# tanwanirahul/surreal

Hardware: AMD Instinct MI355X
Metric: PPO learner env-steps/sec/node (GAE+update) at 1/2/4/8 GPUs; % HBM roofline (higher is better)
Workload: dtype f32; 1 GPU; C3: synthetic PPO learner batch, reference PPO defaults (LSTM 100, horizon 5, heads 300x200, n_step 25, adapt, z-filter, 10/10 epochs), SawyerLift state dims (obs 42, act 8), 1024 segments split over 1 GPU(s) (1024 per GPU); segments_per_gpu=1024, n_step=25, env_steps_per_learn_per_gpu=25600, global_segments=1024, parallelism=single, epochs_run_last=10, ppo_mode=adapt, launch=hipGraph replay

## Files before the change

### include/surreal_mi.h

```cpp
#ifndef SURREAL_MI_H
#define SURREAL_MI_H

#include <stdint.h>

#ifdef __cplusplus
extern "C" {
#endif

#define SMI_OK            0
#define SMI_E_ARG        -1
#define SMI_E_NOFIT      -2
#define SMI_E_LAUNCH     -3

int         smi_version(void);
const char* smi_last_error(void);

const char* smi_last_launch(void);

int64_t smi_workspace_bytes(void);
int     smi_set_workspace(void* dev_ptr, int64_t bytes);
typedef struct smi_context smi_context;
smi_context* smi_context_create(void* workspace, int64_t bytes);
int          smi_context_make_current(smi_context* ctx);
int          smi_context_destroy(smi_context* ctx);

#define SMI_KT_GEMM_FWD    0
#define SMI_KT_GEMM_DX     1
#define SMI_KT_GEMM_DW     2
#define SMI_KT_GEMM_REDUCE 3
#define SMI_KT_LSTM_FWD    4
#define SMI_KT_LSTM_BWD    5
#define SMI_KT_CNN_FWD     6
#define SMI_KT_CNN_BWD     7
#define SMI_KT_GAE         8
#define SMI_KT_POLICY_STATS 9
#define SMI_KT_POLICY_GRAD 10
#define SMI_KT_VALUE_ROWS  11
#define SMI_KT_ADAM        12
#define SMI_KT_ZF_TMAJOR   13
int smi_kernel_timing(int on);
int smi_kernel_timing_report(int cls, double* out4);

int smi_calib_mfma(int n_wg, int iters, float* out, long long* stamps, void* stream);
int smi_calib_stream(const float* x, float* y, int64_t n, void* stream);
int smi_clock_probe(const int* flag, long long max_ticks, long long* out3, void* stream);
int smi_clock_probe_stop(int* flag, int value, void* stream);

int64_t smi_mlp_param_count(int in_dim, int h1, int h2, int out_dim, int with_log_var);

int64_t smi_ppo_fused_lds_bytes(int rows, int obs_dim, int h1, int h2, int act_dim,
                                int critic_h1, int critic_h2);

int64_t smi_ppo_fused_max_params(void);

int smi_zfilter_apply(const float* x, float* out, int64_t rows, int dim,
                      const float* running_sum, const float* running_sumsq,
                      const float* count, float eps, void* stream);

int smi_zfilter_update(const float* x, int64_t rows, int dim, int64_t row_stride,
                       float* running_sum, float* running_sumsq, float* count,
                       void* stream);

int smi_zfilter_colstats(const float* x, int64_t rows, int dim, int64_t row_stride,
                         float* out_sum, float* out_sumsq, void* stream);

int smi_zfilter_tmajor(const float* obs, const float* obs_next, int B, int T, int S, int D,
                       int use_zf, const float* running_sum, const float* running_sumsq,
                       const float* count, float eps, float* out, int ldo, int form,
                       void* stream);

int smi_reward_filter(float* rewards, int64_t n, float reward_scale, int mode,
                      float* running_sum, float* running_sumsq, float* count,
                      float eps, void* stream);

int smi_reward_filter_partial(float* rewards, int64_t n, float reward_scale, int forward,
                              const float* running_sum, const float* running_sumsq,
                              const float* count, float eps, double* sums3, void* stream);
int smi_reward_filter_commit(const double* sums3, float* running_sum, float* running_sumsq,
                             float* count, void* stream);

int smi_diag_gauss(const float* actions, const float* prob0, const float* prob1,
                   int64_t rows, int act_dim,
                   float* loglik, float* lik, float* kl, float* entropy, void* stream);

int smi_mlp_forward(const float* params, int in_dim, int h1, int h2, int out_dim,
                    int out_act, int with_log_var,
                    const float* x, int64_t rows, int64_t row_stride,
                    int use_zf, const float* zf_sum, const float* zf_sumsq,
                    const float* zf_count, float zf_eps,
                    float* out, void* stream);

int smi_head_forward(const float* params, int in_dim, int h1, int h2, int out_dim, int tanh_out,
                     const float* x, int64_t ldx, int64_t rows, float* ha1, float* ha2,
                     float* y, float* wT, void* stream);
int smi_head_backward_input(const float* params, int in_dim, int h1, int h2, int out_dim,
                            const float* wT, const float* dz, int64_t rows, const float* ha1,
                            const float* ha2, float* dh2, float* dh1, int dx0, int dxn, float* dx,
                            int64_t lddx, const float* mask, int64_t ldm, void* stream);

int smi_ppo_critic_gae(const float* critic_params, int obs_dim, int h1, int h2,
                       int use_zf, const float* zf_sum, const float* zf_sumsq,
                       const float* zf_count, float zf_eps,
                       const float* obs, const float* obs_next,
                       const float* rewards, const float* dones, int B, int T,
                       const float* gamma_tab, const float* lam_tab,
                       float gamma, float gamma_T,
                       float* values, float* adv_raw, float* ret, void* stream);

int smi_gae_windows(const float* values, float* values_masked,
                    const float* rewards, const float* dones,
                    int64_t B, int T, int horizon,
                    const float* gamma_tab, const float* lam_tab,
                    float gamma, float gamma_H,
                    float* adv, float* ret, double* adv_partials,
                    int* n_partials, void* stream);
int smi_gae_windows_max_partials(int64_t B, int T);

int smi_moments(const float* x, int64_t n, const double* partials, int n_partials,
                double* out3, void* stream);

typedef struct smi_ppo_args {
  int B;
  int obs_dim, h1, h2, act_dim;
  int critic_h1, critic_h2;
  int epoch_policy, epoch_baseline;
  int mode;
  int norm_adv;
  int clip_actor_grad, clip_critic_grad;
  int use_zf;
  const float* obs;      int64_t obs_stride;
  const float* actions;  int64_t act_stride;
  const float* behave;   int64_t beh_stride;
  const float* adv_raw;
  const double* adv_moments;
  const float* ret;
  const float* zf_sum;  const float* zf_sumsq;  const float* zf_count;
  const float* rzf_sum; const float* rzf_sumsq; const float* rzf_count;
  float zf_eps;
  float* actor;  const float* ref_actor;  float* critic;
  float* actor_m; float* actor_v; float* critic_m; float* critic_v;
  int* actor_step; int* critic_step;
  const float* hyper;
  double kl_target;
  float kl_cutoff_coeff;
  float actor_max_norm, critic_max_norm;
  float actor_wd, critic_wd;
  float beta1, beta2, adam_eps;
  float* stats;
  float* kl_record; int* kl_count; int kl_capacity;
  int64_t B_global;
  float* xbuf;
  int* dp_state;
  float* adv_out;
} smi_ppo_args;

#define SMI_HYP_CLIP_EPS   0
#define SMI_HYP_BETA       1
#define SMI_HYP_LR_ACTOR   2
#define SMI_HYP_LR_CRITIC  3
#define SMI_HYPX_CLIP_LO   4
#define SMI_HYPX_CLIP_HI   5
#define SMI_HYP_COUNT      6

#define SMI_ST_SURR_LOSS        0
#define SMI_ST_CLIP_SURR_LOSS   1
#define SMI_ST_KL_LOSS_ADAPT    2
#define SMI_ST_ENTROPY          3
#define SMI_ST_POL_KL           4
#define SMI_ST_GRAD_NORM_ACTOR  5
#define SMI_ST_VAL_LOSS         6
#define SMI_ST_VAL_EXPL_VAR     7
#define SMI_ST_GRAD_NORM_CRITIC 8
#define SMI_ST_AVG_RETURN       9
#define SMI_ST_AVG_LOG_SIG     10
#define SMI_ST_AVG_BEHAVE_LIK  11
#define SMI_ST_AVG_IS_WEIGHT   12
#define SMI_ST_REF_BEHAVE_DIFF 13
#define SMI_ST_EPOCHS_RUN      14
#define SMI_ST_POL_KL_ADAPT    15
#define SMI_ST_COUNT           16

int smi_ppo_update_fused(const smi_ppo_args* args, void* stream);

int64_t smi_ppo_xbuf_floats(int obs_dim, int h1, int h2, int act_dim, int critic_h1,
                            int critic_h2, int mode);
int smi_ppo_epoch_grad(const smi_ppo_args* args, int epoch, void* stream);
int smi_ppo_epoch_apply(const smi_ppo_args* args, int epoch, void* stream);

#define SMI_RNN_PH_GAE           0
#define SMI_RNN_PH_PREP          1
#define SMI_RNN_PH_POLICY_FWD    2
#define SMI_RNN_PH_POLICY_BWD    3
#define SMI_RNN_PH_POLICY_APPLY  4
#define SMI_RNN_PH_VALUE_GRAD    5
#define SMI_RNN_PH_VALUE_APPLY   6
#define SMI_RNN_PH_ZSTATS        7
#define SMI_RNN_PH_ZAPPLY        8
#define SMI_RNN_PH_POLICY_DECIDE 9

typedef struct smi_ppo_rnn_args {
  int B, T, horizon;
  int obs_dim, rnn_hidden;
  int h1, h2, act_dim;
  int critic_h1, critic_h2;
  int epoch_policy, epoch_baseline;
  int mode, norm_adv, clip_actor_grad, clip_critic_grad, use_zf;
  int64_t B_global;
  const float* obs;
  const float* obs_next;
  const float* actions;
  const float* rewards;
  const float* dones;
  const float* behave;
  const float* h0;
  const float* c0;
  float* lstm; float* actor; float* critic;
  const float* ref_lstm; const float* ref_actor;
  float* zf_sum; float* zf_sumsq; float* zf_count;
  const float* rzf_sum; const float* rzf_sumsq; const float* rzf_count;
  float zf_eps;
  float* actor_m; float* actor_v; float* critic_m; float* critic_v;
  int* actor_step; int* critic_step;
  const float* hyper;
  const float* gamma_tab; const float* lam_tab;
  float gamma, gamma_H;
  double kl_target;
  float kl_cutoff_coeff, actor_max_norm, critic_max_norm, actor_wd, critic_wd;
  float beta1, beta2, adam_eps;
  float* stats;
  float* kl_record; int* kl_count; int kl_capacity;
  double* moments;
  double* pstat;
  float* xbuf;
  double* zbuf;
  void* scratch; int64_t scratch_bytes;
  int pix_c, pix_h, pix_w, cnn_feat;
  const uint8_t* pixels;
  const uint8_t* pixels_next;
  float* adv_out; float* ret_out;
  int rnn_layer;
  int prep_independent;
} smi_ppo_rnn_args;

#define SMI_RNN_PSTAT 16
int64_t smi_ppo_rnn_scratch_bytes(int B, int T, int horizon, int obs_dim, int rnn_hidden,
                                  int h1, int h2, int act_dim, int critic_h1, int critic_h2,
                                  int pix_c, int pix_h, int pix_w, int cnn_feat, int rnn_layer);
int64_t smi_ppo_rnn_xbuf_floats(int obs_dim, int rnn_hidden, int h1, int h2, int act_dim,
                                int critic_h1, int critic_h2, int pix_c, int pix_h, int pix_w,
                                int cnn_feat, int rnn_layer);
int64_t smi_lstm_param_count(int in_dim, int hidden);
int smi_ppo_rnn_phase(const smi_ppo_rnn_args* args, int phase, int epoch, void* stream);

int smi_lstm_forward(const float* xproj, const float* w_hh, const float* b_hh,
                     const float* h0, const float* c0, int S, int B, int H,
                     float* hbuf, float* cbuf, float* gates_act, void* stream);
int smi_lstm_backward(const float* dh, const float* gates_act, const float* cbuf,
                      const float* w_hh, int S, int B, int H, float* dgates, void* stream);
int smi_lstm_forward_x(const float* x, int64_t ldx, int din, const float* w_ih,
                       const float* b_ih, const float* w_hh, const float* b_hh,
                       const float* h0, const float* c0, int S, int B, int H, float* hbuf,
                       float* cbuf, float* gates_act, float* xproj_scratch, void* stream);

int64_t smi_cnn_param_count(int C, int H, int W, int F);
int64_t smi_cnn_scratch_bytes(int64_t rows, int C, int H, int W, int F);
int smi_cnn_forward(const float* params, const uint8_t* pix, const uint8_t* pix_next, int64_t B,
                    int64_t T, int64_t rows, int C, int H, int W, int F, float* a1, float* a2,
                    float* feat, int64_t ldf, void* stream);
int smi_cnn_backward(const float* params, const uint8_t* pix, const uint8_t* pix_next, int64_t B,
                     int64_t T, int64_t rows, int C, int H, int W, int F, const float* a1,
                     const float* a2, const float* dz, int64_t lddz, float* grad, void* scratch,
                     int64_t scratch_bytes, void* stream);

int smi_zfilter_accumulate(const float* sum_in, const float* sumsq_in, int dim, float rows,
                           float* running_sum, float* running_sumsq, float* count,
                           void* stream);

int smi_adam_clip(float* params, const float* grad, float* m, float* v, int64_t n,
                  int* step, const float* lr_ptr, float beta1, float beta2,
                  float eps, float weight_decay, float max_norm, float clip_value,
                  const int* skip_flag, float* norm_out, void* stream);

int smi_linear_forward(const float* x, int64_t ldx, int rows, int in_dim, const float* w,
                       int64_t ldw, const float* b, int out_dim, int act, float* y, int64_t ldy,
                       void* stream);
int smi_linear_backward_input(const float* dy, int64_t ldg, int rows, int out_dim,
                              const float* w, int64_t ldw, int in_dim, const float* relu_mask,
                              int64_t ldm, float* dx, int64_t lddx, void* stream);
int smi_linear_forward_cat(const float* x, int64_t ldx, int rows, int in_dim, const float* w,
                           int64_t ldw, const float* b, int out_dim, int act, float* y,
                           int64_t ldy, const float* s, int64_t lds, int s_cols, void* stream);
int smi_linear_backward_weight(const float* dy, int64_t ldg, int rows, int out_dim,
                               const float* x, int64_t ldx, int in_dim, float* dw, int64_t lddw,
                               float* db, int accumulate, void* stream);
int smi_dw_group_begin(void);
int smi_dw_group_flush(void* stream);

int smi_mse_grad(const float* q, int64_t q_stride, const float* y, int64_t n, float* dq,
                 float* loss, void* stream);
int smi_neg_mean_grad(const float* q, int64_t q_stride, int64_t n, float* dq, float* loss,
                      void* stream);
int smi_tanh_backward(const float* dy, int64_t ldg, const float* y, int64_t ldy, int64_t rows,
                      int cols, float* dz, int64_t ldz, void* stream);
int smi_copy_cols(const float* src, int64_t lds, int64_t rows, int cols, float* dst,
                  int64_t ldd, void* stream);
int smi_layernorm_forward(const float* x, int64_t ldx, int64_t rows, int n, const float* gamma,
                          const float* beta, float eps, float* y, int64_t ldy, float* mean,
                          float* rstd, void* stream);
int smi_layernorm_backward(const float* dy, int64_t ldg, const float* x, int64_t ldx,
                           const float* mean, const float* rstd, const float* gamma, int64_t rows,
                           int n, int relu_input, float* dx, int64_t lddx, float* dgamma,
                           float* dbeta, void* stream);

int smi_mlp3_forward_stacked(const float* params, int64_t pstride, const int64_t* offsets6,
                             int in_dim, int h1, int h2, int out_dim, int out_act, const float* x,
                             int64_t ldx, int n, float* y, int64_t ldy, void* stream);

int smi_copy_to_host(void* host_dst, const void* src, int64_t nbytes, void* stream);
int smi_copy_gather(void* dst, const void* const* srcs, const int64_t* dst_offsets,
                    const int64_t* nbytes, int n, void* stream);
int smi_soft_update(float* target, const float* src, int64_t n, float tau, void* stream);
int smi_ddpg_stats(const float* actions, int64_t lda, int act_dim, const float* rewards,
                   int64_t rs, const float* y, const float* q, int64_t qs, int64_t n,
                   float* stats4, void* stream);

int smi_ddpg_target(const float* rewards, const float* dones, const float* q_next,
                    const float* q_next2, int64_t n, float gamma_n, float* y,
                    void* stream);

int smi_mt_seed(uint64_t seed, uint32_t* host_state625);
int smi_mt_randint_host(uint32_t* host_state625, int64_t n, int64_t batch,
                        int64_t* out);
int smi_mt_randint(uint32_t* dev_state625, int64_t n, int64_t batch,
                   int64_t* out_indices, void* stream);

int smi_gather_rows(const float* table, int64_t cols, const int64_t* idx,
                    int64_t batch, float* out, void* stream);

#ifdef __cplusplus
}
#endif
#endif
```

### surreal_amd/_lib.py

```python
import contextlib
import threading
import ctypes
import gc
import os

import torch

HERE = os.path.dirname(os.path.abspath(__file__))
_VARIANT = os.environ.get('SMI_LIB_VARIANT')
LIB_PATH = os.path.join(HERE, 'libsurreal_mi.so' if not _VARIANT else f'libsurreal_mi_{_VARIANT}.so')

c_int, c_i64, c_f32, c_f64, c_vp = ctypes.c_int, ctypes.c_int64, ctypes.c_float, ctypes.c_double, ctypes.c_void_p
P = ctypes.c_void_p

HYP_CLIP_EPS, HYP_BETA, HYP_LR_ACTOR, HYP_LR_CRITIC, HYP_CLIP_LO, HYP_CLIP_HI, HYP_COUNT = range(7)
ST_NAMES = ['_surr_loss', '_clip_surr_loss', '_kl_loss_adapt', '_entropy', '_pol_kl',
            'grad_norm_actor', '_val_loss', '_val_explained_var', 'grad_norm_critic',
            '_avg_return_targ', '_avg_log_sig', '_avg_behave_likelihood', '_avg_is_weight',
            '_ref_behave_diff', 'epochs_run', '_pol_kl_adapt']
ST_COUNT = len(ST_NAMES)
ST = {n: i for i, n in enumerate(ST_NAMES)}


class PPOArgs(ctypes.Structure):
    _fields_ = [
        ('B', c_int), ('obs_dim', c_int), ('h1', c_int), ('h2', c_int), ('act_dim', c_int),
        ('critic_h1', c_int), ('critic_h2', c_int),
        ('epoch_policy', c_int), ('epoch_baseline', c_int),
        ('mode', c_int), ('norm_adv', c_int),
        ('clip_actor_grad', c_int), ('clip_critic_grad', c_int), ('use_zf', c_int),
        ('obs', P), ('obs_stride', c_i64),
        ('actions', P), ('act_stride', c_i64),
        ('behave', P), ('beh_stride', c_i64),
        ('adv_raw', P), ('adv_moments', P), ('ret', P),
        ('zf_sum', P), ('zf_sumsq', P), ('zf_count', P),
        ('rzf_sum', P), ('rzf_sumsq', P), ('rzf_count', P),
        ('zf_eps', c_f32),
        ('actor', P), ('ref_actor', P), ('critic', P),
        ('actor_m', P), ('actor_v', P), ('critic_m', P), ('critic_v', P),
        ('actor_step', P), ('critic_step', P),
        ('hyper', P),
        ('kl_target', c_f64), ('kl_cutoff_coeff', c_f32),
        ('actor_max_norm', c_f32), ('critic_max_norm', c_f32),
        ('actor_wd', c_f32), ('critic_wd', c_f32),
        ('beta1', c_f32), ('beta2', c_f32), ('adam_eps', c_f32),
        ('stats', P),
        ('kl_record', P), ('kl_count', P), ('kl_capacity', c_int),
        ('B_global', c_i64), ('xbuf', P), ('dp_state', P),
        ('adv_out', P),
    ]


class RNNArgs(ctypes.Structure):
    _fields_ = [
        ('B', c_int), ('T', c_int), ('horizon', c_int), ('obs_dim', c_int), ('rnn_hidden', c_int),
        ('h1', c_int), ('h2', c_int), ('act_dim', c_int), ('critic_h1', c_int), ('critic_h2', c_int),
        ('epoch_policy', c_int), ('epoch_baseline', c_int),
        ('mode', c_int), ('norm_adv', c_int), ('clip_actor_grad', c_int), ('clip_critic_grad', c_int),
        ('use_zf', c_int),
        ('B_global', c_i64),
        ('obs', P), ('obs_next', P), ('actions', P), ('rewards', P), ('dones', P), ('behave', P),
        ('h0', P), ('c0', P),
        ('lstm', P), ('actor', P), ('critic', P), ('ref_lstm', P), ('ref_actor', P),
        ('zf_sum', P), ('zf_sumsq', P), ('zf_count', P),
        ('rzf_sum', P), ('rzf_sumsq', P), ('rzf_count', P),
        ('zf_eps', c_f32),
        ('actor_m', P), ('actor_v', P), ('critic_m', P), ('critic_v', P),
        ('actor_step', P), ('critic_step', P),
        ('hyper', P), ('gamma_tab', P), ('lam_tab', P),
        ('gamma', c_f32), ('gamma_H', c_f32),
        ('kl_target', c_f64),
        ('kl_cutoff_coeff', c_f32), ('actor_max_norm', c_f32), ('critic_max_norm', c_f32),
        ('actor_wd', c_f32), ('critic_wd', c_f32),
        ('beta1', c_f32), ('beta2', c_f32), ('adam_eps', c_f32),
        ('stats', P), ('kl_record', P), ('kl_count', P), ('kl_capacity', c_int),
        ('moments', P), ('pstat', P), ('xbuf', P), ('zbuf', P),
        ('scratch', P), ('scratch_bytes', c_i64),
        ('pix_c', c_int), ('pix_h', c_int), ('pix_w', c_int), ('cnn_feat', c_int),
        ('pixels', P), ('pixels_next', P),
        ('adv_out', P), ('ret_out', P),
        ('rnn_layer', c_int), ('prep_independent', c_int),
    ]


RNN_PH_GAE, RNN_PH_PREP, RNN_PH_POLICY_FWD, RNN_PH_POLICY_BWD, RNN_PH_POLICY_APPLY, \
    RNN_PH_VALUE_GRAD, RNN_PH_VALUE_APPLY, RNN_PH_ZSTATS, RNN_PH_ZAPPLY, RNN_PH_POLICY_DECIDE = range(10)
RNN_PSTAT = 16
KT_NAMES = ['gemm_fwd', 'gemm_dx', 'gemm_dw', 'gemm_splitk_reduce', 'lstm_fwd', 'lstm_bwd',
            'cnn_fwd', 'cnn_bwd',
            'gae', 'policy_rows_stats', 'policy_rows_grad', 'value_rows', 'adam', 'zf_tmajor']
KT_BYTES = set(KT_NAMES[8:])


def kernel_timing(on):
    check(lib().smi_kernel_timing(1 if on else 0), 'smi_kernel_timing')


def kernel_timing_report():
    out = {}
    buf = (c_f64 * 4)()
    for i, n in enumerate(KT_NAMES):
        check(lib().smi_kernel_timing_report(i, ctypes.cast(buf, P)), 'smi_kernel_timing_report')
        if buf[0] > 0:
            out[n] = (int(buf[0]), float(buf[1]), float(buf[2]))
    return out

_SIGS = {
    'smi_version': (c_int, []),
    'smi_last_error': (ctypes.c_char_p, []),
    'smi_last_launch': (ctypes.c_char_p, []),
    'smi_workspace_bytes': (c_i64, []),
    'smi_set_workspace': (c_int, [P, c_i64]),
    'smi_context_create': (P, [P, c_i64]),
    'smi_context_make_current': (c_int, [P]),
    'smi_context_destroy': (c_int, [P]),
    'smi_mlp_param_count': (c_i64, [c_int, c_int, c_int, c_int, c_int]),
    'smi_ppo_fused_lds_bytes': (c_i64, [c_int] * 7),
    'smi_ppo_fused_max_params': (c_i64, []),
    'smi_zfilter_apply': (c_int, [P, P, c_i64, c_int, P, P, P, c_f32, P]),
    'smi_zfilter_update': (c_int, [P, c_i64, c_int, c_i64, P, P, P, P]),
    'smi_zfilter_colstats': (c_int, [P, c_i64, c_int, c_i64, P, P, P]),
    'smi_zfilter_tmajor': (c_int, [P, P, c_int, c_int, c_int, c_int, c_int, P, P, P, c_f32, P,
                                   c_int, c_int, P]),
    'smi_reward_filter': (c_int, [P, c_i64, c_f32, c_int, P, P, P, c_f32, P]),
    'smi_reward_filter_partial': (c_int, [P, c_i64, c_f32, c_int, P, P, P, c_f32, P, P]),
    'smi_reward_filter_commit': (c_int, [P, P, P, P, P]),
    'smi_dw_group_begin': (c_int, []),
    'smi_dw_group_flush': (c_int, [P]),
    'smi_layernorm_forward': (c_int, [P, c_i64, c_i64, c_int, P, P, c_f32, P, c_i64, P, P, P]),
    'smi_layernorm_backward': (c_int, [P, c_i64, P, c_i64, P, P, P, c_i64, c_int, c_int, P, c_i64,
                                       P, P, P]),
    'smi_diag_gauss': (c_int, [P, P, P, c_i64, c_int, P, P, P, P, P]),
    'smi_mlp_forward': (c_int, [P, c_int, c_int, c_int, c_int, c_int, c_int, P, c_i64, c_i64,
                                c_int, P, P, P, c_f32, P, P]),
    'smi_ppo_critic_gae': (c_int, [P, c_int, c_int, c_int, c_int, P, P, P, c_f32, P, P, P, P,
                                   c_int, c_int, P, P, c_f32, c_f32, P, P, P, P]),
    'smi_gae_windows': (c_int, [P, P, P, P, c_i64, c_int, c_int, P, P, c_f32, c_f32, P, P, P,
                                P, P]),
    'smi_gae_windows_max_partials': (c_int, [c_i64, c_int]),
    'smi_moments': (c_int, [P, c_i64, P, c_int, P, P]),
    'smi_ppo_update_fused': (c_int, [ctypes.POINTER(PPOArgs), P]),
    'smi_ppo_xbuf_floats': (c_i64, [c_int] * 7),
    'smi_ppo_epoch_grad': (c_int, [ctypes.POINTER(PPOArgs), c_int, P]),
    'smi_ppo_epoch_apply': (c_int, [ctypes.POINTER(PPOArgs), c_int, P]),
    'smi_zfilter_accumulate': (c_int, [P, P, c_int, c_f32, P, P, P, P]),
    'smi_adam_clip': (c_int, [P, P, P, P, c_i64, P, P, c_f32, c_f32, c_f32, c_f32, c_f32, c_f32,
                              P, P, P]),
    'smi_linear_forward': (c_int, [P, c_i64, c_int, c_int, P, c_i64, P, c_int, c_int, P, c_i64, P]),
    'smi_linear_forward_cat': (c_int, [P, c_i64, c_int, c_int, P, c_i64, P, c_int, c_int, P, c_i64,
                                       P, c_i64, c_int, P]),
    'smi_linear_backward_input': (c_int, [P, c_i64, c_int, c_int, P, c_i64, c_int, P, c_i64, P,
                                          c_i64, P]),
    'smi_linear_backward_weight': (c_int, [P, c_i64, c_int, c_int, P, c_i64, c_int, P, c_i64, P,
                                           c_int, P]),
    'smi_mse_grad': (c_int, [P, c_i64, P, c_i64, P, P, P]),
    'smi_neg_mean_grad': (c_int, [P, c_i64, c_i64, P, P, P]),
    'smi_tanh_backward': (c_int, [P, c_i64, P, c_i64, c_i64, c_int, P, c_i64, P]),
    'smi_copy_cols': (c_int, [P, c_i64, c_i64, c_int, P, c_i64, P]),
    'smi_mlp3_forward_stacked': (c_int, [P, c_i64, P, c_int, c_int, c_int, c_int, c_int, P, c_i64,
                                         c_int, P, c_i64, P]),
    'smi_copy_to_host': (c_int, [P, P, c_i64, P]),
    'smi_copy_gather': (c_int, [P, P, P, P, c_int, P]),
    'smi_head_forward': (c_int, [P, c_int, c_int, c_int, c_int, c_int, P, c_i64, c_i64, P, P, P, P,
                                 P]),
    'smi_head_backward_input': (c_int, [P, c_int, c_int, c_int, c_int, P, P, c_i64, P, P, P, P,
                                        c_int, c_int, P, c_i64, P, c_i64, P]),
    'smi_soft_update': (c_int, [P, P, c_i64, c_f32, P]),
    'smi_ddpg_stats': (c_int, [P, c_i64, c_int, P, c_i64, P, P, c_i64, c_i64, P, P]),
    'smi_ddpg_target': (c_int, [P, P, P, P, c_i64, c_f32, P, P]),
    'smi_mt_seed': (c_int, [ctypes.c_uint64, P]),
    'smi_mt_randint_host': (c_int, [P, c_i64, c_i64, P]),
    'smi_mt_randint': (c_int, [P, c_i64, c_i64, P, P]),
    'smi_gather_rows': (c_int, [P, c_i64, P, c_i64, P, P]),
    'smi_lstm_param_count': (c_i64, [c_int, c_int]),
    'smi_kernel_timing': (c_int, [c_int]),
    'smi_kernel_timing_report': (c_int, [c_int, P]),
    'smi_calib_mfma': (c_int, [c_int, c_int, P, P, P]),
    'smi_calib_stream': (c_int, [P, P, c_i64, P]),
    'smi_clock_probe': (c_int, [P, ctypes.c_longlong, P, P]),
    'smi_clock_probe_stop': (c_int, [P, c_int, P]),
    'smi_ppo_rnn_scratch_bytes': (c_i64, [c_int] * 15),
    'smi_ppo_rnn_xbuf_floats': (c_i64, [c_int] * 12),
    'smi_cnn_param_count': (c_i64, [c_int] * 4),
    'smi_cnn_scratch_bytes': (c_i64, [c_i64] + [c_int] * 4),
    'smi_cnn_forward': (c_int, [P, P, P, c_i64, c_i64, c_i64] + [c_int] * 4 + [P, P, P, c_i64, P]),
    'smi_cnn_backward': (c_int, [P, P, P, c_i64, c_i64, c_i64] + [c_int] * 4 +
                         [P, P, P, c_i64, P, P, c_i64, P]),
    'smi_ppo_rnn_phase': (c_int, [ctypes.POINTER(RNNArgs), c_int, c_int, P]),
    'smi_lstm_forward': (c_int, [P, P, P, P, P, c_int, c_int, c_int, P, P, P, P]),
    'smi_lstm_backward': (c_int, [P, P, P, P, c_int, c_int, c_int, P, P]),
    'smi_lstm_forward_x': (c_int, [P, c_i64, c_int, P, P, P, P, P, P, c_int, c_int, c_int,
                                   P, P, P, P, P]),
}

_lib = None


def lib():
    global _lib
    if _lib is None:
        if not os.path.exists(LIB_PATH):
            raise RuntimeError('libsurreal_mi.so not built: run `python -c "import __graft_entry__ as '
                               'g; g.build()"` (no CPU fallback exists)')
        L = ctypes.CDLL(LIB_PATH)
        for name, (res, args) in _SIGS.items():
            fn = getattr(L, name)
            fn.restype = res
            fn.argtypes = args
        _lib = L
    return _lib


def exported_symbols():
    return list(_SIGS)


def check(rc, name):
    if rc != 0:
        msg = lib().smi_last_error().decode(errors='replace')
        raise RuntimeError(f'{name} failed (rc={rc}): {msg}')


def call(name, *args):
    rc = getattr(lib(), name)(*args)
    check(rc, name)
    return rc


def ptr(t):
    if t is None:
        return None
    if not t.is_cuda:
        raise RuntimeError('surreal_amd kernels take device (HIP) tensors; got a CPU tensor '
                           '(there is no CPU fallback)')
    return ctypes.c_void_p(t.data_ptr())


def stream(device=None):
    return ctypes.c_void_p(torch.cuda.current_stream(device).cuda_stream)


_workspaces = {}


def ensure_workspace(device):
    dev = torch.device(device)
    key = dev.index if dev.index is not None else torch.cuda.current_device()
    if key not in _workspaces:
        nbytes = lib().smi_workspace_bytes()
        ws = torch.zeros(nbytes // 4, dtype=torch.float32, device=dev)
        _workspaces[key] = ws
        check(lib().smi_set_workspace(ctypes.c_void_p(ws.data_ptr()), nbytes), 'smi_set_workspace')
    return _workspaces[key]


_ctx_tls = threading.local()


class Context(object):

    def __init__(self, device):
        self.device = torch.device(device)
        nbytes = lib().smi_workspace_bytes()
        self.ws = torch.zeros(nbytes // 4, dtype=torch.float32, device=self.device)
        self.handle = lib().smi_context_create(ctypes.c_void_p(self.ws.data_ptr()), nbytes)
        if not self.handle:
            check(-1, 'smi_context_create')

    def make_current(self):
        check(lib().smi_context_make_current(ctypes.c_void_p(self.handle)), 'smi_context_make_current')
        _ctx_tls.current = self

    def __del__(self):
        h, self.handle = getattr(self, 'handle', None), None
        if h and _lib is not None:
            _lib.smi_context_destroy(ctypes.c_void_p(h))


@contextlib.contextmanager
def gc_paused():
    was = gc.isenabled()
    gc.disable()
    try:
        yield
    finally:
        if was:
            gc.enable()


def require_gpu():
    if not torch.cuda.is_available():
        raise RuntimeError('surreal_amd requires an AMD GPU (HIP); none is visible and there is '
                           'no CPU fallback')
```

### surreal_amd/csrc/linear_kernels.hip

```cpp
#include <cmath>
#include <algorithm>
#include <stdlib.h>
#include <type_traits>
#include "smi_device.hpp"
#include "smi_internal.hpp"
#include "lstm_cell.hpp"

namespace smi {

enum { EPI_FWD = 0, EPI_DX = 1, EPI_DW = 2 };

constexpr int GBM = 64, GBN = 64, GBK = 32;
constexpr int LD_KC = 36;
constexpr int LD_RC = 80;
constexpr int G_STAGE = 2560;

struct GemmArgs {
  int M, N, K;
  const float* A; int64_t a_rs, a_cs;
  const float* B; int64_t b_rs, b_cs;
  float* C; int64_t ldc;
  const float* bias;
  int act;
  const float* mask; int64_t ldm;
  int accumulate;
  int ones_col;
  float* bias_out;
  int kchunk;
  float* part;
  const int* skip;
  int avec, bvec;
  const float* B2; int64_t b2_rs; int split_col, c1_real;
  float* C2; int64_t ldc2; float* bias_out2;
  const float* xsrc; int64_t xlds; int xcols;
};

__device__ __forceinline__ float dw_put(const GemmArgs& g, int m, int n, float v) {
  if (n == g.ones_col) {
    const float b = g.accumulate ? g.bias_out[m] + v : v;
    g.bias_out[m] = b;
    if (g.bias_out2) {
      const float b2 = g.accumulate ? g.bias_out2[m] + v : v;
      g.bias_out2[m] = b2;
      return b * b + b2 * b2;
    }
    return b * b;
  }
  float* dst;
  if (g.B2 && n >= g.split_col) dst = g.C2 + (int64_t)m * g.ldc2 + (n - g.split_col);
  else if (g.B2 && n >= g.c1_real) return 0.f;
  else dst = g.C + (int64_t)m * g.ldc + n;
  const float r = g.accumulate ? *dst + v : v;
  *dst = r;
  return r * r;
}

struct TileRegs { float v[8]; };

struct TileIdx { int mt, nt, z; };
__device__ __forceinline__ TileIdx gemm_tile_index() {
  const int gm = gridDim.x, gn = gridDim.y;
  const int nwg = gm * gn * gridDim.z;
  const int orig = blockIdx.x + gm * (blockIdx.y + gn * blockIdx.z);
  int w = orig;
  if (nwg > 8) {
    const int x = orig & 7, q = nwg >> 3, r = nwg & 7;
    w = (x < r ? x * (q + 1) : r * (q + 1) + (x - r) * q) + (orig >> 3);
  }
  TileIdx t;
  t.nt = w % gn;
  t.mt = (w / gn) % gm;
  t.z = w / (gn * gm);
  return t;
}

template <bool KCONTIG>
__device__ __forceinline__ void gemm_load(const float* __restrict__ P, int64_t rs, int64_t cs,
                                          int r0, int rdata, int k0, int kmax, int ones_col,
                                          bool vec, TileRegs& t) {
  if (vec && ones_col < 0 && r0 + 64 <= rdata && k0 + 32 <= kmax) {
    const float* base = KCONTIG ? P + (int64_t)r0 * rs + k0 : P + (int64_t)k0 * cs + r0;
#pragma unroll
    for (int j = 0; j < 2; ++j) {
      const int q = threadIdx.x + j * kWG;
      const float* src = KCONTIG ? base + (int64_t)(q >> 3) * rs + ((q & 7) << 2)
                                 : base + (int64_t)(q >> 4) * cs + ((q & 15) << 2);
      const float4 x = *reinterpret_cast<const float4*>(src);
      t.v[4 * j + 0] = x.x; t.v[4 * j + 1] = x.y; t.v[4 * j + 2] = x.z; t.v[4 * j + 3] = x.w;
    }
    return;
  }
  if (vec) {
#pragma unroll
    for (int j = 0; j < 2; ++j) {
      const int q = threadIdx.x + j * kWG;
      if (KCONTIG) {
        const int r = q >> 3, k = (q & 7) << 2;
        const int rr = r0 + r, kk = k0 + k;
        const int rc = rr < rdata ? rr : rdata - 1;
        const int kc = kk < kmax ? kk : kmax - 4;
        const float4 x = *reinterpret_cast<const float4*>(P + (int64_t)rc * rs + kc);
        const bool ok = rr < rdata && kk < kmax;
        t.v[4 * j + 0] = ok ? x.x : 0.f; t.v[4 * j + 1] = ok ? x.y : 0.f;
        t.v[4 * j + 2] = ok ? x.z : 0.f; t.v[4 * j + 3] = ok ? x.w : 0.f;
      } else {
        const int k = q >> 4, r = (q & 15) << 2;
        const int rr = r0 + r, kk = k0 + k;
        const int rc = rr < rdata ? rr : rdata - 4;
        const int kc = kk < kmax ? kk : kmax - 1;
        const float4 x = *reinterpret_cast<const float4*>(P + (int64_t)kc * cs + rc);
        const bool okk = kk < kmax, ok = okk && rr < rdata;
        t.v[4 * j + 0] = ok ? x.x : 0.f; t.v[4 * j + 1] = ok ? x.y : 0.f;
        t.v[4 * j + 2] = ok ? x.z : 0.f; t.v[4 * j + 3] = ok ? x.w : 0.f;
        if (ones_col >= 0 && okk) {
#pragma unroll
          for (int e = 0; e < 4; ++e)
            if (rr + e == ones_col) t.v[4 * j + e] = 1.f;
        }
      }
    }
    return;
  }
#pragma unroll
  for (int j = 0; j < 8; ++j) {
    const int idx = threadIdx.x + j * kWG;
    const int r = KCONTIG ? (idx >> 5) : (idx & 63);
    const int k = KCONTIG ? (idx & 31) : (idx >> 6);
    const int rr = r0 + r, kk = k0 + k;
    const int rc = rr < rdata ? rr : rdata - 1;
    const int kc = kk < kmax ? kk : kmax - 1;
    const float x = P[(int64_t)rc * rs + (int64_t)kc * cs];
    t.v[j] = (rr < rdata && kk < kmax) ? x : 0.f;
    if (ones_col >= 0 && rr == ones_col && kk < kmax) t.v[j] = 1.f;
  }
}

template <bool KCONTIG>
__device__ __forceinline__ void gemm_store(float* __restrict__ S, bool vec, const TileRegs& t) {
  if (vec) {
#pragma unroll
    for (int j = 0; j < 2; ++j) {
      const int q = threadIdx.x + j * kWG;
      const float4 x = float4{t.v[4 * j], t.v[4 * j + 1], t.v[4 * j + 2], t.v[4 * j + 3]};
      if (KCONTIG) {
        const int r = q >> 3, k = (q & 7) << 2;
        *reinterpret_cast<float4*>(S + r * LD_KC + k) = x;
      } else {
        const int k = q >> 4, r = (q & 15) << 2;
        *reinterpret_cast<float4*>(S + k * LD_RC + r) = x;
      }
    }
    return;
  }
#pragma unroll
  for (int j = 0; j < 8; ++j) {
    const int idx = threadIdx.x + j * kWG;
    const int r = KCONTIG ? (idx >> 5) : (idx & 63);
    const int k = KCONTIG ? (idx & 31) : (idx >> 6);
    if (KCONTIG) S[r * LD_KC + k] = t.v[j];
    else S[k * LD_RC + r] = t.v[j];
  }
}

template <int EPI, bool AK, bool BK>
__global__ void __launch_bounds__(kWG)
gemm_kernel(GemmArgs g) {
  if (g.skip && g.skip[0] != 0) return;
  __shared__ __attribute__((aligned(16))) float sA[2][G_STAGE];
  __shared__ __attribute__((aligned(16))) float sB[2][G_STAGE];
  const int tid = threadIdx.x, lane = tid & 63, wave = tid >> 6;
  const int li = lane & 15, lk = lane >> 4;
  const TileIdx ti = gemm_tile_index();
  const int m0 = ti.mt * GBM, n0 = ti.nt * GBN;
  const int kb = ti.z * g.kchunk;
  const int ke = min(g.K, kb + g.kchunk);
  const int nk = (ke - kb + GBK - 1) / GBK;
  f32x4 tot[4];
#pragma unroll
  for (int c = 0; c < 4; ++c) tot[c] = f32x4{0.f, 0.f, 0.f, 0.f};
  TileRegs ra[2], rb[2];
  const int bdata = g.ones_col >= 0 ? g.ones_col : g.N;
  if (nk > 0) {
    gemm_load<AK>(g.A, g.a_rs, g.a_cs, m0, g.M, kb, ke, -1, g.avec, ra[0]);
    gemm_load<BK>(g.B, g.b_cs, g.b_rs, n0, bdata, kb, ke, g.ones_col, g.bvec, rb[0]);
  }
  if (nk > 1) {
    gemm_load<AK>(g.A, g.a_rs, g.a_cs, m0, g.M, kb + GBK, ke, -1, g.avec, ra[1]);
    gemm_load<BK>(g.B, g.b_cs, g.b_rs, n0, bdata, kb + GBK, ke, g.ones_col, g.bvec, rb[1]);
  }
  if (nk > 0) {
    gemm_store<AK>(sA[0], g.avec, ra[0]);
    gemm_store<BK>(sB[0], g.bvec, rb[0]);
  }
  __syncthreads();
  const int ar = wave * 16 + li;
  auto kstep = [&](int kt, auto cur_c) {
    constexpr int cur = decltype(cur_c)::value;
    if (kt + 2 < nk) {
      gemm_load<AK>(g.A, g.a_rs, g.a_cs, m0, g.M, kb + (kt + 2) * GBK, ke, -1, g.avec, ra[cur]);
      gemm_load<BK>(g.B, g.b_cs, g.b_rs, n0, bdata, kb + (kt + 2) * GBK, ke, g.ones_col, g.bvec,
                    rb[cur]);
    }
    const float* As = sA[cur];
    const float* Bs = sB[cur];
    f32x4 acc[4];
#pragma unroll
    for (int c = 0; c < 4; ++c) acc[c] = f32x4{0.f, 0.f, 0.f, 0.f};
    float av[8], bv[4][8];
#pragma unroll
    for (int u = 0; u < 8; ++u) {
      const int k = 4 * u + lk;
      av[u] = AK ? As[ar * LD_KC + k] : As[k * LD_RC + ar];
#pragma unroll
      for (int c = 0; c < 4; ++c) {
        const int n = c * 16 + li;
        bv[c][u] = BK ? Bs[n * LD_KC + k] : Bs[k * LD_RC + n];
      }
    }
#pragma unroll
    for (int u = 0; u < 8; ++u)
#pragma unroll
      for (int c = 0; c < 4; ++c) acc[c] = mfma4(av[u], bv[c][u], acc[c]);
#pragma unroll
    for (int c = 0; c < 4; ++c) tot[c] += acc[c];
    if (kt + 1 < nk) {
      gemm_store<AK>(sA[cur ^ 1], g.avec, ra[cur ^ 1]);
      gemm_store<BK>(sB[cur ^ 1], g.bvec, rb[cur ^ 1]);
    }
    __syncthreads();
  };
  for (int kt = 0; kt < nk; kt += 2) {
    kstep(kt, std::integral_constant<int, 0>{});
    if (kt + 1 < nk) kstep(kt + 1, std::integral_constant<int, 1>{});
  }
#pragma unroll
  for (int c = 0; c < 4; ++c) {
    const int n = n0 + c * 16 + li;
    if (n >= g.N) continue;
    float bias_n = 0.f;
    if constexpr (EPI == EPI_FWD) bias_n = g.bias ? g.bias[n] : 0.f;
#pragma unroll
    for (int i = 0; i < 4; ++i) {
      const int m = m0 + wave * 16 + lk * 4 + i;
      if (m >= g.M) continue;
      float v = tot[c][i];
      if constexpr (EPI == EPI_FWD) {
        if (g.part) {
          g.part[((int64_t)ti.z * g.M + m) * g.N + n] = v;
          continue;
        }
        v += bias_n;
        if (g.act == ACT_RELU) v = v > 0.f ? v : 0.f;
        else if (g.act == ACT_TANH) v = tanhf(v);
        g.C[(int64_t)m * g.ldc + n] = v;
      } else if constexpr (EPI == EPI_DX) {
        if (g.part) {
          g.part[((int64_t)ti.z * g.M + m) * g.N + n] = v;
          continue;
        }
        if (g.mask) v = g.mask[(int64_t)m * g.ldm + n] > 0.f ? v : 0.f;
        g.C[(int64_t)m * g.ldc + n] = v;
      } else {
        if (g.part) {
          g.part[((int64_t)ti.z * g.M + m) * g.N + n] = v;
        } else if (n == g.ones_col) {
          g.bias_out[m] = g.accumulate ? g.bias_out[m] + v : v;
        } else {
          float* dst = g.C + (int64_t)m * g.ldc + n;
          *dst = g.accumulate ? *dst + v : v;
        }
      }
    }
  }
}

constexpr int DWD_ZMAX = 8192;
__device__ __attribute__((aligned(16))) float g_dwd_zero[DWD_ZMAX];
__device__ __attribute__((aligned(16))) float g_dwd_one[4] = {1.f, 0.f, 0.f, 0.f};

__global__ void __launch_bounds__(kWG)
gemm_splitk_reduce_kernel(const float* __restrict__ part, int S, GemmArgs g, const float* bias,
                          int act, const float* mask) {
  if (g.skip && g.skip[0] != 0) return;
  __shared__ float red[4][64];
  const int M = g.M, N = g.N;
  const int64_t MN = (int64_t)M * N;
  const int el = threadIdx.x & 63, zl = threadIdx.x >> 6;
  const int64_t e = (int64_t)blockIdx.x * 64 + el;
  const int64_t ec = e < MN ? e : MN - 1;
  float s0 = 0.f, s1 = 0.f, s2 = 0.f, s3 = 0.f;
  int z = zl;
  if (S <= 64) {
    const float* pz = part + (int64_t)zl * MN + ec;
    const int64_t st4 = 4 * MN;
    float v[16];
#pragma unroll
    for (int k = 0; k < 16; ++k) v[k] = *(zl + 4 * k < S ? pz + k * st4 : g_dwd_zero);
#pragma unroll
    for (int k = 0; k < 16; ++k) asm volatile("" : "+v"(v[k]));
    const int nfull = S > zl + 12 ? (S - zl - 12 + 15) / 16 : 0;
#pragma unroll
    for (int j = 0; j < 4; ++j) {
      if (j < nfull) {
        s0 += v[4 * j]; s1 += v[4 * j + 1]; s2 += v[4 * j + 2]; s3 += v[4 * j + 3];
      }
    }
#pragma unroll
    for (int k = 0; k < 16; ++k)
      if (k >= 4 * nfull && zl + 4 * k < S) s0 += v[k];
    z = S;
  }
  for (; z + 12 < S; z += 16) {
    s0 += part[(int64_t)z * MN + ec];
    s1 += part[(int64_t)(z + 4) * MN + ec];
    s2 += part[(int64_t)(z + 8) * MN + ec];
    s3 += part[(int64_t)(z + 12) * MN + ec];
  }
  for (; z < S; z += 4) s0 += part[(int64_t)z * MN + ec];
  red[zl][el] = (s0 + s1) + (s2 + s3);
  __syncthreads();
  if (zl != 0 || e >= MN) return;
  float s = (red[0][el] + red[1][el]) + (red[2][el] + red[3][el]);
  const int m = (int)(e / N), n = (int)(e - (int64_t)m * N);
  if (bias) s += bias[n];
  if (act == ACT_RELU) s = s > 0.f ? s : 0.f;
  else if (act == ACT_TANH) s = tanhf(s);
  if (mask && !(mask[(int64_t)m * g.ldm + n] > 0.f)) s = 0.f;
  dw_put(g, m, n, s);
}

template <int NKU>
__global__ void __launch_bounds__(kWG)
gemm_smallk_fwd_kernel(const float* __restrict__ X, int64_t ldx, int M, int K,
                       const float* __restrict__ W, int64_t ldw, const float* __restrict__ bias,
                       int N, int act, float* __restrict__ Y, int64_t ldy, const int* skip) {
  if (skip && skip[0] != 0) return;
  extern __shared__ __attribute__((aligned(16))) float sW[];
  constexpr int LDK = 4 * NKU + 1;
  constexpr int LDO = 68;
  float* sb = sW + N * LDK;
  float* so = sb + ((N + 3) & ~3) + (threadIdx.x >> 6) * 16 * LDO;
  {
    const int tot = N * LDK;
    for (int e0 = threadIdx.x; e0 < tot; e0 += 8 * kWG) {
      float v[8];
#pragma unroll
      for (int j = 0; j < 8; ++j) {
        const int e = e0 + j * kWG;
        const int ec = e < tot ? e : tot - 1;
        const int n = ec / LDK, k = ec - n * LDK;
        const float x = W[(int64_t)n * ldw + (k < K ? k : K - 1)];
        v[j] = k < K ? x : 0.f;
      }
#pragma unroll
      for (int j = 0; j < 8; ++j) {
        const int e = e0 + j * kWG;
        if (e < tot) sW[e] = v[j];
      }
    }
  }
  for (int n = threadIdx.x; n < N; n += kWG) sb[n] = bias ? bias[n] : 0.f;
  __syncthreads();
  const int lane = threadIdx.x & 63, wave = threadIdx.x >> 6, li = lane & 15, lk = lane >> 4;
  const bool vec_out = ((reinterpret_cast<uintptr_t>(Y) & 15) == 0) && (ldy % 4 == 0);
  for (int tile = blockIdx.x; tile * 64 < M; tile += gridDim.x) {
    const int m = tile * 64 + wave * 16 + li;
    const int mc = m < M ? m : M - 1;
    float a[NKU];
#pragma unroll
    for (int u = 0; u < NKU; ++u) {
      const int k = 4 * u + lk;
      const float x = X[(int64_t)mc * ldx + (k < K ? k : K - 1)];
      a[u] = k < K ? x : 0.f;
    }
    for (int nb = 0; nb < N; nb += 64) {
      f32x4 acc[4];
      const float* w[4];
#pragma unroll
      for (int c = 0; c < 4; ++c) {
        acc[c] = f32x4{0.f, 0.f, 0.f, 0.f};
        const int n = nb + c * 16 + li;
        w[c] = sW + (n < N ? n : N - 1) * LDK + lk;
      }
      float bw[4][NKU];
#pragma unroll
      for (int c = 0; c < 4; ++c)
#pragma unroll
        for (int u = 0; u < NKU; ++u) bw[c][u] = w[c][4 * u];
#pragma unroll
      for (int u = 0; u < NKU; ++u)
#pragma unroll
        for (int c = 0; c < 4; ++c) acc[c] = mfma4(a[u], bw[c][u], acc[c]);
#pragma unroll
      for (int c = 0; c < 4; ++c) {
        const int col = nb + c * 16 + li;
        const float bn = col < N ? sb[col] : 0.f;
#pragma unroll
        for (int i = 0; i < 4; ++i) {
          float v = acc[c][i] + bn;
          if (act == ACT_RELU) v = v > 0.f ? v : 0.f;
          else if (act == ACT_TANH) v = tanhf(v);
          so[(lk * 4 + i) * LDO + c * 16 + li] = v;
        }
      }
      __builtin_amdgcn_wave_barrier();
#pragma unroll
      for (int j = 0; j < 4; ++j) {
        const int r = j * 4 + (lane >> 4), c4 = (lane & 15) * 4;
        const int row = tile * 64 + wave * 16 + r, col = nb + c4;
        const float4 v = *reinterpret_cast<const float4*>(so + r * LDO + c4);
        if (row < M) {
          float* dst = Y + (int64_t)row * ldy + col;
          if (vec_out && col + 3 < N) {
            *reinterpret_cast<float4*>(dst) = v;
          } else {
            if (col < N) dst[0] = v.x;
            if (col + 1 < N) dst[1] = v.y;
            if (col + 2 < N) dst[2] = v.z;
            if (col + 3 < N) dst[3] = v.w;
          }
        }
      }
      __builtin_amdgcn_wave_barrier();
    }
  }
}

static int launch_smallk_fwd(const float* X, int64_t ldx, int M, int K, const float* W,
                             int64_t ldw, const float* b, int N, int act, float* Y, int64_t ldy,
                             hipStream_t st, const int* skip) {
  const int nku = (K + 3) / 4 <= 4 ? 4 : (K + 3) / 4 <= 8 ? 8 : (K + 3) / 4 <= 12 ? 12 : 16;
  const size_t lds = ((size_t)N * (4 * nku + 1) + ((N + 3) & ~3) + 4 * 16 * 68) * 4;
  const int tiles = (M + 63) / 64;
  const int kslot = ktime_begin(st);
  const char* form = "gemm_smallk_fwd_kernel";
#define SMI_SK_CASE(V)                                                                         \
  if (nku == V) {                                                                              \
    form = "gemm_smallk_fwd_kernel<" #V ">";                                                   \
    auto k = gemm_smallk_fwd_kernel<V>;                                                        \
    allow_lds(k, lds);                                                                         \
    static int cap = 0;                                                                        \
    if (!cap) cap = resident_grid(k, kWG, lds);                                                \
    const int grid = tiles < cap ? tiles : cap;                                                \
    hipLaunchKernelGGL(k, dim3(grid), dim3(kWG), lds, st, X, ldx, M, K, W, ldw, b, N, act, Y, \
                       ldy, skip);                                                             \
  }
  SMI_SK_CASE(4) SMI_SK_CASE(8) SMI_SK_CASE(12) SMI_SK_CASE(16)
#undef SMI_SK_CASE
  ktime_end(kslot, KT_GEMM_FWD, 2.0 * M * (double)N * K, st);
  return check_launch(form);
}

constexpr int D2_T = 128, D2_LD = 144;

__device__ __forceinline__ void dw2_load(const float* __restrict__ P, int64_t rs, int c0,
                                         int cdata, int ones_col, int k0, int kmax, float4 (&r)[4]) {
#pragma unroll
  for (int j = 0; j < 4; ++j) {
    const int q = threadIdx.x + j * kWG;
    const int k = q >> 5, c = c0 + ((q & 31) << 2);
    const int kk = k0 + k;
    const int kc = kk < kmax ? kk : kmax - 1;
    const int cc = c + 3 < cdata ? c : (cdata >= 4 ? cdata - 4 : 0);
    float4 v = *reinterpret_cast<const float4*>(P + (int64_t)kc * rs + cc);
    const bool okk = kk < kmax;
    v.x = okk && c < cdata ? v.x : 0.f;
    v.y = okk && c + 1 < cdata ? v.y : 0.f;
    v.z = okk && c + 2 < cdata ? v.z : 0.f;
    v.w = okk && c + 3 < cdata ? v.w : 0.f;
    if (ones_col >= 0 && okk) {
      if (c == ones_col) v.x = 1.f;
      if (c + 1 == ones_col) v.y = 1.f;
      if (c + 2 == ones_col) v.z = 1.f;
      if (c + 3 == ones_col) v.w = 1.f;
    }
    r[j] = v;
  }
}

__device__ __forceinline__ void dw2_store(float* __restrict__ S, const float4 (&r)[4]) {
#pragma unroll
  for (int j = 0; j < 4; ++j) {
    const int q = threadIdx.x + j * kWG;
    *reinterpret_cast<float4*>(S + (q >> 5) * D2_LD + ((q & 31) << 2)) = r[j];
  }
}

__global__ void __launch_bounds__(kWG)
gemm_dw128_kernel(GemmArgs g) {
  if (g.skip && g.skip[0] != 0) return;
  __shared__ __attribute__((aligned(16))) float sA[2][32 * D2_LD];
  __shared__ __attribute__((aligned(16))) float sB[2][32 * D2_LD];
  const int tid = threadIdx.x, lane = tid & 63, wave = tid >> 6;
  const int li = lane & 15, lk = lane >> 4;
  const TileIdx ti = gemm_tile_index();
  const int m0 = ti.mt * D2_T, n0 = ti.nt * D2_T;
  const int kb = ti.z * g.kchunk;
  const int ke = min(g.K, kb + g.kchunk);
  const int nk = (ke - kb + 31) / 32;
  const int bdata = g.ones_col >= 0 ? g.ones_col + 1 : g.N;
  const int bload = g.ones_col >= 0 ? g.ones_col : g.N;
  f32x4 acc[2][8];
#pragma unroll
  for (int a = 0; a < 2; ++a)
#pragma unroll
    for (int b = 0; b < 8; ++b) acc[a][b] = f32x4{0.f, 0.f, 0.f, 0.f};
  float4 ra[4], rb[4];
  (void)bdata;
  if (nk > 0) {
    dw2_load(g.A, g.a_cs, m0, g.M, -1, kb, ke, ra);
    dw2_load(g.B, g.b_rs, n0, bload, g.ones_col, kb, ke, rb);
    dw2_store(sA[0], ra);
    dw2_store(sB[0], rb);
  }
  __syncthreads();
  for (int kt = 0; kt < nk; ++kt) {
    const int cur = kt & 1;
    if (kt + 1 < nk) {
      dw2_load(g.A, g.a_cs, m0, g.M, -1, kb + (kt + 1) * 32, ke, ra);
      dw2_load(g.B, g.b_rs, n0, bload, g.ones_col, kb + (kt + 1) * 32, ke, rb);
    }
    const float* As = sA[cur];
    const float* Bs = sB[cur];
#pragma unroll
    for (int u = 0; u < 8; ++u) {
      const int kr = (4 * u + lk) * D2_LD;
      float av[2], bv[8];
#pragma unroll
      for (int a = 0; a < 2; ++a) av[a] = As[kr + wave * 32 + a * 16 + li];
#pragma unroll
      for (int b = 0; b < 8; ++b) bv[b] = Bs[kr + b * 16 + li];
#pragma unroll
      for (int a = 0; a < 2; ++a)
#pragma unroll
        for (int b = 0; b < 8; ++b) acc[a][b] = mfma4(av[a], bv[b], acc[a][b]);
    }
    if (kt + 1 < nk) {
      dw2_store(sA[cur ^ 1], ra);
      dw2_store(sB[cur ^ 1], rb);
    }
    __syncthreads();
  }
#pragma unroll
  for (int b = 0; b < 8; ++b) {
    const int n = n0 + b * 16 + li;
    if (n >= g.N) continue;
#pragma unroll
    for (int a = 0; a < 2; ++a)
#pragma unroll
      for (int i = 0; i < 4; ++i) {
        const int m = m0 + wave * 32 + a * 16 + lk * 4 + i;
        if (m >= g.M) continue;
        const float v = acc[a][b][i];
        if (g.part) {
          g.part[((int64_t)ti.z * g.M + m) * g.N + n] = v;
        } else if (n == g.ones_col) {
          g.bias_out[m] = g.accumulate ? g.bias_out[m] + v : v;
        } else {
          float* dst = g.C + (int64_t)m * g.ldc + n;
          *dst = g.accumulate ? *dst + v : v;
        }
      }
  }
}

#ifndef SMI_DWD_DIAG
#define SMI_DWD_DIAG 0
#endif
#ifndef SMI_DWD_TRACE
#define SMI_DWD_TRACE (SMI_DWD_DIAG == 3)
#endif
#ifndef SMI_DWD_P
#define SMI_DWD_P 4
#endif
#ifndef SMI_DWD_OCC
#define SMI_DWD_OCC 2
#endif
constexpr int DWD_P = SMI_DWD_P;


template <int MT, int NT, bool VA, bool VB, int NB = NT>
__device__ __forceinline__ void dwd_load(const GemmArgs& g, int r, int ke, int m0, int n0, int bdata,
                                         float (&av)[MT], float (&bv)[NT]) {
  const int li = threadIdx.x & 15;
  const bool ok = r < ke;
  const float* Ar = ok ? g.A + (int64_t)r * g.a_cs : g_dwd_zero;
  const float* Br = ok ? g.B + (int64_t)r * g.b_rs : g_dwd_zero;
  const float* Br2 = g.B2 ? (ok ? g.B2 + (int64_t)r * g.b2_rs - g.split_col
                                : g_dwd_zero - g.split_col)
                          : Br;
  const int split = g.B2 ? g.split_col : 0x7fffffff;
  const float* one = ok ? g_dwd_one : g_dwd_zero;
  if constexpr (MT == 4 && VA) {
    const int c = min(m0 + 4 * li, g.M - 4);
    const float4 x = *reinterpret_cast<const float4*>(Ar + c);
    av[0] = x.x; av[1] = x.y; av[2] = x.z; av[3] = x.w;
  } else {
#pragma unroll
    for (int t = 0; t < MT; ++t) av[t] = Ar[min(m0 + MT * li + t, g.M - 1)];
  }
#pragma unroll
  for (int h = 0; h < NB / 4; ++h) {
    const int cb = n0 + 64 * h + 4 * li;
    if constexpr (VB) {
      const float* src = cb < bdata ? (cb >= split ? Br2 : Br) + cb
                                    : (cb == g.ones_col ? one : g_dwd_zero);
      const float4 x = *reinterpret_cast<const float4*>(src);
      bv[4 * h] = x.x; bv[4 * h + 1] = x.y; bv[4 * h + 2] = x.z; bv[4 * h + 3] = x.w;
    } else {
#pragma unroll
      for (int t = 0; t < 4; ++t) {
        const int c = cb + t;
        bv[4 * h + t] = *(c < bdata ? (c >= split ? Br2 : Br) + c
                                    : (c == g.ones_col ? one : g_dwd_zero));
      }
    }
  }
}

#ifndef SMI_DWD_FAST
#define SMI_DWD_FAST 1
#endif
__device__ __forceinline__ bool use_dwd_fast() { return SMI_DWD_FAST != 0; }

template <int MT, int NT, int NB, int RS>
__device__ __forceinline__ void dwd_main_fast(const GemmArgs& g, int rw, int nsteps, int m0, int n0,
                                              int bdata, f32x4 (&acc)[MT][NT]) {
  static_assert(MT == 4 || MT == 1, "fast dW loop: 4 m sub-tiles (float4 A) or 1 (scalar A)");
  constexpr int NH = NB / 4;
  const int li = threadIdx.x & 15;
  const float* pa = g.A + (int64_t)rw * g.a_cs + (MT == 4 ? min(m0 + 4 * li, g.M - 4)
                                                          : min(m0 + li, g.M - 1));
  const int64_t sa = (int64_t)RS * g.a_cs;
  const float* pb[NH];
  int64_t sb[NH];
#pragma unroll
  for (int h = 0; h < NH; ++h) {
    const int cb = n0 + 64 * h + 4 * li;
    if (cb < bdata) {
      if (g.B2 && cb >= g.split_col) {
        pb[h] = g.B2 + (int64_t)rw * g.b2_rs + (cb - g.split_col);
        sb[h] = (int64_t)RS * g.b2_rs;
      } else {
        pb[h] = g.B + (int64_t)rw * g.b_rs + cb;
        sb[h] = (int64_t)RS * g.b_rs;
      }
    } else {
      pb[h] = cb == g.ones_col ? g_dwd_one : g_dwd_zero;
      sb[h] = 0;
    }
  }
  float4 av[DWD_P], bv[DWD_P][NH];
  using gf4 = const __attribute__((address_space(1))) f32x4;
  using gf1 = const __attribute__((address_space(1))) float;
  auto f4 = [](const f32x4 x) { return float4{x[0], x[1], x[2], x[3]}; };
  auto load = [&](int p) {
    if constexpr (MT == 4) av[p] = f4(*(gf4*)pa);
    else av[p].x = *(gf1*)pa;
    pa += sa;
#pragma unroll
    for (int h = 0; h < NH; ++h) {
      bv[p][h] = f4(*(gf4*)pb[h]);
      pb[h] += sb[h];
    }
  };
  auto step = [&](int p) {
    const float a4[4] = {av[p].x, av[p].y, av[p].z, av[p].w};
#if SMI_DWD_DIAG == 2
    acc[0][0][0] += (a4[0] + a4[1]) + (a4[2] + a4[3]);
#pragma unroll
    for (int h = 0; h < NH; ++h) acc[0][0][1] += (bv[p][h].x + bv[p][h].y) + (bv[p][h].z + bv[p][h].w);
#else
#pragma unroll
    for (int b = 0; b < NB; ++b) {
      const float4 q = bv[p][b >> 2];
      const float bb = (b & 3) == 0 ? q.x : (b & 3) == 1 ? q.y : (b & 3) == 2 ? q.z : q.w;
#pragma unroll
      for (int a = 0; a < MT; ++a) acc[a][b] = mfma4(a4[a], bb, acc[a][b]);
    }
#endif
  };
#pragma unroll
  for (int p = 0; p < DWD_P; ++p) {
    load(p);
    __builtin_amdgcn_sched_barrier(0);
  }
  f32x4 tot[MT][NT];
  if constexpr (MT == 1) {
#pragma unroll
    for (int b = 0; b < NT; ++b) tot[0][b] = f32x4{0.f, 0.f, 0.f, 0.f};
  }
  for (int s0 = DWD_P; s0 < nsteps; s0 += DWD_P) {
#pragma unroll
    for (int p = 0; p < DWD_P; ++p) {
      step(p);
      if constexpr (SMI_DWD_DIAG != 1) load(p);
      __builtin_amdgcn_sched_barrier(0);
    }
    if constexpr (MT == 1) {
#pragma unroll
      for (int b = 0; b < NB; ++b) {
        tot[0][b] += acc[0][b];
        acc[0][b] = f32x4{0.f, 0.f, 0.f, 0.f};
      }
    }
  }
#pragma unroll
  for (int p = 0; p < DWD_P; ++p) step(p);
  if constexpr (MT == 1) {
#pragma unroll
    for (int b = 0; b < NB; ++b) acc[0][b] = tot[0][b] + acc[0][b];
  }
}

template <int MT, int NT, bool VA, bool VB, int WV>
__device__ __forceinline__ void dwd_tile(const GemmArgs& g, const TileIdx ti, float4* dwd_red) {
  const int lane = threadIdx.x & 63, wave = threadIdx.x >> 6;
  const int li = lane & 15, lk = lane >> 4;
  const int m0 = ti.mt * 16 * MT, n0 = ti.nt * 16 * NT;
  const int kb = ti.z * g.kchunk;
  const int ke = min(g.K, kb + g.kchunk);
  constexpr int RS = 4 * WV;
  const int nsteps = (ke - kb + RS - 1) / RS;
  const int bdata = g.ones_col >= 0 ? g.ones_col : g.N;
  const int rw = kb + 4 * wave + lk;
  f32x4 acc[MT][NT];
#pragma unroll
  for (int a = 0; a < MT; ++a)
#pragma unroll
    for (int b = 0; b < NT; ++b) acc[a][b] = f32x4{0.f, 0.f, 0.f, 0.f};
  auto mainloop = [&](auto nbc) {
    constexpr int NB = decltype(nbc)::value;
    float av[DWD_P][MT], bv[DWD_P][NT];
#pragma unroll
    for (int p = 0; p < DWD_P; ++p)
      dwd_load<MT, NT, VA, VB, NB>(g, rw + RS * p, ke, m0, n0, bdata, av[p], bv[p]);
    for (int s0 = 0; s0 < nsteps; s0 += DWD_P) {
#pragma unroll
      for (int p = 0; p < DWD_P; ++p) {
#pragma unroll
        for (int b = 0; b < NB; ++b)
#pragma unroll
          for (int a = 0; a < MT; ++a) acc[a][b] = mfma4(av[p][a], bv[p][b], acc[a][b]);
        dwd_load<MT, NT, VA, VB, NB>(g, rw + RS * (s0 + p + DWD_P), ke, m0, n0, bdata, av[p], bv[p]);
        __builtin_amdgcn_sched_barrier(0);
      }
    }
  };
  constexpr bool kFast = VB && ((VA && MT == 4) || MT == 1);
  bool fast = false;
  if constexpr (kFast)
    fast = use_dwd_fast() && nsteps >= DWD_P && nsteps % DWD_P == 0 && kb + nsteps * RS <= ke;
  constexpr int NBH = NT > 4 ? 4 : NT;
  if (NT == 8 && n0 + 64 >= g.N) {
    if constexpr (kFast) {
      if (fast) dwd_main_fast<MT, NT, NBH, RS>(g, rw, nsteps, m0, n0, bdata, acc);
      else mainloop(std::integral_constant<int, NBH>{});
    } else {
      mainloop(std::integral_constant<int, NBH>{});
    }
  } else {
    if constexpr (kFast) {
      if (fast) dwd_main_fast<MT, NT, NT, RS>(g, rw, nsteps, m0, n0, bdata, acc);
      else mainloop(std::integral_constant<int, NT>{});
    } else {
      mainloop(std::integral_constant<int, NT>{});
    }
  }
  auto put = [&](float4* buf) {
#pragma unroll
    for (int a = 0; a < MT; ++a)
#pragma unroll
      for (int b = 0; b < NT; ++b) {
        const f32x4 v = acc[a][b];
        buf[(a * NT + b) * 64 + lane] = float4{v[0], v[1], v[2], v[3]};
      }
  };
  auto add = [&](const float4* buf) {
#pragma unroll
    for (int a = 0; a < MT; ++a)
#pragma unroll
      for (int b = 0; b < NT; ++b) {
        const float4 v = buf[(a * NT + b) * 64 + lane];
        acc[a][b] += f32x4{v.x, v.y, v.z, v.w};
      }
  };
#pragma unroll
  for (int h = WV / 2; h >= 1; h >>= 1) {
#pragma unroll
    for (int c = 0; c < h; c += 2) {
      if (wave >= h + c && wave < h + c + 2) put(dwd_red + (wave - h - c) * MT * NT * 64);
      __syncthreads();
      if (wave >= c && wave < c + 2 && wave < h) add(dwd_red + (wave - c) * MT * NT * 64);
      __syncthreads();
    }
  }
  if (wave != 0) return;
  const bool vec_part = g.part && (g.N & 3) == 0;
#pragma unroll
  for (int a = 0; a < MT; ++a)
#pragma unroll
    for (int i = 0; i < 4; ++i) {
      const int m = m0 + MT * (lk * 4 + i) + a;
      if (m >= g.M) continue;
#pragma unroll
      for (int h = 0; h < NT / 4; ++h) {
        const int nb = n0 + 64 * h + 4 * li;
        if (vec_part) {
          if (nb < g.N)
            *reinterpret_cast<float4*>(g.part + ((int64_t)ti.z * g.M + m) * g.N + nb) =
                float4{acc[a][4 * h][i], acc[a][4 * h + 1][i], acc[a][4 * h + 2][i],
                       acc[a][4 * h + 3][i]};
          continue;
        }
#pragma unroll
        for (int t = 0; t < 4; ++t) {
          const int n = nb + t;
          if (n >= g.N) continue;
          const float v = acc[a][4 * h + t][i];
          if (g.part) g.part[((int64_t)ti.z * g.M + m) * g.N + n] = v;
          else dw_put(g, m, n, v);
        }
      }
    }
}

template <int MT, int NT, bool VA, bool VB, int WV>
__global__ void __launch_bounds__(64 * WV, WV == 4 ? SMI_DWD_OCC : 1)
gemm_dwd_kernel(GemmArgs g) {
  if (g.skip && g.skip[0] != 0) return;
  extern __shared__ float4 dwd_red[];
  dwd_tile<MT, NT, VA, VB, WV>(g, gemm_tile_index(), dwd_red);
}

constexpr int kDwGroupMax = 8;
constexpr int kDwSplitMax = 6;
struct DwGroup {
  DwEpilogue x;
  GemmArgs g[kDwGroupMax];
  int wg0[kDwGroupMax + 1];
  int rb0[kDwGroupMax + 1];
  int gm[kDwGroupMax], gn[kDwGroupMax], S[kDwGroupMax];
  int vec[kDwGroupMax];
  int narrow[kDwGroupMax];
  int n;
};

#ifndef SMI_DWG_NT
#define SMI_DWG_NT 4
#endif
#ifndef SMI_DWG_OCC
#define SMI_DWG_OCC (SMI_DWG_NT == 4 ? 3 : 2)
#endif
constexpr int DWG_NT = SMI_DWG_NT;

#if SMI_DWD_TRACE
constexpr int kDwTraceMax = 8192;
__device__ unsigned long long g_dw_trace[kDwTraceMax][6];
extern "C" int smi_diag_dw_trace(void* dst, int n) {
  if (n > kDwTraceMax) n = kDwTraceMax;
  return hipMemcpyFromSymbol(dst, HIP_SYMBOL(g_dw_trace), (size_t)n * 48, 0, hipMemcpyDeviceToHost) == hipSuccess ? n : -1;
}
#endif

template <int WV>
__device__ __forceinline__ void dwd_group_run(const DwGroup& G, int orig, int nwg, float4* dwd_red,
                                              int& gi, int& rows) {
  int w = orig;
  if (nwg > 8) {
    const int x = orig & 7, q = nwg >> 3, r = nwg & 7;
    w = (x < r ? x * (q + 1) : r * (q + 1) + (x - r) * q) + (orig >> 3);
  }
  gi = 0;
  while (gi + 1 < G.n && w >= G.wg0[gi + 1]) ++gi;
  const GemmArgs& g = G.g[gi];
  if (g.skip && g.skip[0] != 0) return;
  const int local = w - G.wg0[gi], gn = G.gn[gi], gm = G.gm[gi];
  TileIdx ti;
  ti.nt = local % gn;
  ti.mt = (local / gn) % gm;
  ti.z = local / (gn * gm);
  rows = (min(g.K, (ti.z + 1) * g.kchunk) - ti.z * g.kchunk) |
         ((G.narrow[gi] && ti.mt == gm - 1) << 16) | (G.vec[gi] << 17);
  if (G.narrow[gi] && ti.mt == gm - 1) {
    ti.mt *= 4;
    if (G.vec[gi] & 1) dwd_tile<1, DWG_NT, false, true, WV>(g, ti, dwd_red);
    else dwd_tile<1, DWG_NT, false, false, WV>(g, ti, dwd_red);
    return;
  }
  switch (G.vec[gi]) {
    case 3: dwd_tile<4, DWG_NT, true, true, WV>(g, ti, dwd_red); break;
    case 2: dwd_tile<4, DWG_NT, true, false, WV>(g, ti, dwd_red); break;
    case 1: dwd_tile<4, DWG_NT, false, true, WV>(g, ti, dwd_red); break;
    default: dwd_tile<4, DWG_NT, false, false, WV>(g, ti, dwd_red); break;
  }
}

template <int WV>
__global__ void __launch_bounds__(64 * WV, WV == 4 ? SMI_DWG_OCC : 1)
gemm_dwd_group_kernel(DwGroup G) {
  extern __shared__ float4 dwd_red[];
  int gi = 0, rows = 0;
#if SMI_DWD_TRACE
  const unsigned long long t_start = wall_clock64(), c_start = clock64();
#endif
  dwd_group_run<WV>(G, blockIdx.x, gridDim.x, dwd_red, gi, rows);
#if SMI_DWD_TRACE
  __syncthreads();
  if (threadIdx.x == 0 && blockIdx.x < kDwTraceMax) {
    g_dw_trace[blockIdx.x][0] = t_start;
    g_dw_trace[blockIdx.x][1] = wall_clock64();
    g_dw_trace[blockIdx.x][2] = __builtin_amdgcn_s_getreg((31 << 11) | 4);
    g_dw_trace[blockIdx.x][3] = __builtin_amdgcn_s_getreg((31 << 11) | 20) | (gi << 8) |
                                ((unsigned long long)rows << 16);
    g_dw_trace[blockIdx.x][4] = c_start;
    g_dw_trace[blockIdx.x][5] = clock64();
  }
#else
  (void)gi; (void)rows;
#endif
}

template <int BR, bool STG>
__global__ void __launch_bounds__(kVT, 1)
lstm_bwd_dw_kernel(LstmBwdArgs la, DwGroup G) {
  extern __shared__ float4 dwd_red[];
  if ((int)blockIdx.x < la.B) {
    lstm_bwd_q_body<BR, SMI_BPTT_CH4 != 0, STG>(la, blockIdx.x, reinterpret_cast<float*>(dwd_red));
    return;
  }
  int gi = 0, rows = 0;
  dwd_group_run<8>(G, blockIdx.x - la.B, gridDim.x - la.B, dwd_red, gi, rows);
}

__device__ void dw_epilogue_block(const DwEpilogue& x, int nsq) {
  __shared__ double red[kWG / 64];
  const int lane = threadIdx.x & 63, wave = threadIdx.x >> 6;
  float q = 0.f;
  if (x.lvpart) {
    constexpr int NW = kWG / 64;
    for (int j0 = wave; j0 < x.lv_A; j0 += 2 * NW) {
      const int jj[2] = {j0, min(j0 + NW, x.lv_A - 1)};
      float t[2] = {0.f, 0.f};
      int i = lane;
      for (; i + 15 * 64 < x.lv_nb; i += 16 * 64) {
        float v[2][16];
#pragma unroll
        for (int c = 0; c < 2; ++c)
#pragma unroll
          for (int k = 0; k < 16; ++k) v[c][k] = x.lvpart[(int64_t)(i + 64 * k) * x.lv_A + jj[c]];
#pragma unroll
        for (int c = 0; c < 2; ++c)
#pragma unroll
          for (int k = 0; k < 16; ++k) t[c] += v[c][k];
      }
      {
        float v[2][16];
#pragma unroll
        for (int c = 0; c < 2; ++c)
#pragma unroll
          for (int k = 0; k < 16; ++k) {
            const int ik = i + 64 * k;
            v[c][k] = *(ik < x.lv_nb ? x.lvpart + (int64_t)ik * x.lv_A + jj[c] : g_dwd_zero);
          }
#pragma unroll
        for (int c = 0; c < 2; ++c)
#pragma unroll
          for (int k = 0; k < 16; ++k) asm volatile("" : "+v"(v[c][k]));
#pragma unroll
        for (int c = 0; c < 2; ++c)
#pragma unroll
          for (int k = 0; k < 16; ++k)
            if (i + 64 * k < x.lv_nb) t[c] += v[c][k];
      }
      const float e0 = expf(x.lv[jj[0]]), e1 = expf(x.lv[jj[1]]);
      const float g0 = wave_sum(t[0]) * e0;
      const float g1 = wave_sum(t[1]) * e1;
      if (lane == 0) {
        x.lv_out[jj[0]] = g0;
        q += g0 * g0;
        if (j0 + NW < x.lv_A) {
          x.lv_out[jj[1]] = g1;
          q += g1 * g1;
        }
      }
    }
  }
  if (!x.sq) {
    if (threadIdx.x == 0 && x.step) x.step[0] += 1;
    if (threadIdx.x == 0 && x.runs) x.runs[0] += 1;
    return;
  }
  const double t = block_sum_d((double)q, red);
  if (threadIdx.x == 0) {
    x.sq[nsq] = t;
    x.np[0] = nsq + 1;
    if (x.step) x.step[0] += 1;
    if (x.runs) x.runs[0] += 1;
  }
}

template <int U>
__device__ __forceinline__ void red_slabs(const float* const (&p)[U], int64_t MN, int S, int zl,
                                          float (&r)[U]) {
  float s0[U], s1[U], s2[U], s3[U];
#pragma unroll
  for (int u = 0; u < U; ++u) s0[u] = s1[u] = s2[u] = s3[u] = 0.f;
  int z = zl;
  if (S <= 64) {
    const int64_t st4 = 4 * MN;
    float v[U][16];
#pragma unroll
    for (int u = 0; u < U; ++u) {
      const float* pz = p[u] + (int64_t)zl * MN;
#pragma unroll
      for (int k = 0; k < 16; ++k) v[u][k] = *(zl + 4 * k < S ? pz + k * st4 : g_dwd_zero);
    }
#pragma unroll
    for (int u = 0; u < U; ++u)
#pragma unroll
      for (int k = 0; k < 16; ++k) asm volatile("" : "+v"(v[u][k]));
    const int nfull = S > zl + 12 ? (S - zl - 12 + 15) / 16 : 0;
#pragma unroll
    for (int u = 0; u < U; ++u) {
#pragma unroll
      for (int j = 0; j < 4; ++j) {
        if (j < nfull) {
          s0[u] += v[u][4 * j]; s1[u] += v[u][4 * j + 1]; s2[u] += v[u][4 * j + 2]; s3[u] += v[u][4 * j + 3];
        }
      }
#pragma unroll
      for (int k = 0; k < 16; ++k)
        if (k >= 4 * nfull && zl + 4 * k < S) s0[u] += v[u][k];
    }
    z = S;
  }
  for (; z + 12 < S; z += 16) {
#pragma unroll
    for (int u = 0; u < U; ++u) {
      s0[u] += p[u][(int64_t)z * MN];
      s1[u] += p[u][(int64_t)(z + 4) * MN];
      s2[u] += p[u][(int64_t)(z + 8) * MN];
      s3[u] += p[u][(int64_t)(z + 12) * MN];
    }
  }
  for (; z < S; z += 4)
#pragma unroll
    for (int u = 0; u < U; ++u) s0[u] += p[u][(int64_t)z * MN];
#pragma unroll
  for (int u = 0; u < U; ++u) r[u] = (s0[u] + s1[u]) + (s2[u] + s3[u]);
}

template <int U>
__global__ void __launch_bounds__(kWG)
gemm_group_reduce_kernel(DwGroup G) {
  __shared__ float red[4][64 * U];
  __shared__ double sqr[kWG / 64];
  const int ep = G.x.on ? 1 : 0;
  if (ep && blockIdx.x == 0) {
    if (G.x.skip && G.x.skip[0] != 0) return;
    dw_epilogue_block(G.x, G.rb0[G.n]);
    return;
  }
  const int b = (int)blockIdx.x - ep;
  int gi = 0;
  while (gi + 1 < G.n && b >= G.rb0[gi + 1]) ++gi;
  const GemmArgs& g = G.g[gi];
  if (g.skip && g.skip[0] != 0) return;
  const int S = G.S[gi];
  const int64_t MN = (int64_t)g.M * g.N;
  const int el = threadIdx.x & 63, zl = threadIdx.x >> 6;
  const int64_t eb = (int64_t)(b - G.rb0[gi]) * 64 * U;
  const float* p[U];
#pragma unroll
  for (int u = 0; u < U; ++u) p[u] = g.part + min(eb + el + 64 * u, MN - 1);
  float r[U];
  red_slabs<U>(p, MN, S, zl, r);
#pragma unroll
  for (int u = 0; u < U; ++u) red[zl][el + 64 * u] = r[u];
  __syncthreads();
  float q = 0.f;
  for (int i = threadIdx.x; i < 64 * U; i += kWG) {
    const int64_t e = eb + i;
    if (e < MN) {
      const float v = (red[0][i] + red[1][i]) + (red[2][i] + red[3][i]);
      const int m = (int)(e / g.N), n = (int)(e - (int64_t)m * g.N);
      q += dw_put(g, m, n, v);
    }
  }
  if (!G.x.sq) return;
  const double t = block_sum_d((double)q, sqr);
  if (threadIdx.x == 0) G.x.sq[b] = t;
}


constexpr int PN_LD = 20;

template <int EPI, int NTW>
__global__ void __launch_bounds__(kWG)
gemm_panel_kernel(GemmArgs g) {
  if (g.skip && g.skip[0] != 0) return;
  constexpr int NB = 16 * NTW;
  constexpr int BQ = (4 * NB + kWG - 1) / kWG;
  __shared__ __attribute__((aligned(16))) float sB[2][NB * PN_LD + 4];
  const int tid = threadIdx.x, lane = tid & 63, wave = tid >> 6;
  const int li = lane & 15, lk = lane >> 4;
  const TileIdx ti = gemm_tile_index();
  const int r0 = ti.mt * 64 + wave * 16;
  const int n0 = ti.nt * NB;
  const int nch = (g.K + 15) >> 4;
  const float* arow = g.A + (int64_t)min(r0 + li, g.M - 1) * g.a_rs;
  auto load_a = [&](int c) -> float4 {
    const int k = c * 16 + 4 * lk;
    return *reinterpret_cast<const float4*>(k < g.K ? arow + k : g_dwd_zero);
  };
  auto load_b = [&](int c, int q) -> float4 {
    const int idx = tid + q * kWG;
    const float* src;
    if constexpr (EPI == EPI_FWD) {
      const int n = idx >> 2, k = c * 16 + ((idx & 3) << 2);
      const int nc = min(n0 + n, g.N - 1);
      src = (idx < 4 * NB && k < g.K) ? g.B + (int64_t)nc * g.b_cs + k : g_dwd_zero;
    } else {
      const int k = idx / (NB / 4), nq = (idx - k * (NB / 4)) << 2;
      const int kk = c * 16 + k;
      const int nc = min(n0 + nq, g.N - 4);
      src = (idx < 4 * NB && kk < g.K) ? g.B + (int64_t)kk * g.b_rs + nc : g_dwd_zero;
    }
    return *reinterpret_cast<const float4*>(src);
  };
  auto store_b = [&](float* S, int q, float4 r) {
    const int idx = tid + q * kWG;
    const bool ok = idx < 4 * NB;
    if constexpr (EPI == EPI_FWD) {
      const int n = idx >> 2, kq = (idx & 3) << 2;
      *reinterpret_cast<float4*>(S + (ok ? n * PN_LD + kq : NB * PN_LD)) = r;
    } else {
      const int k = idx / (NB / 4), nq = (idx - k * (NB / 4)) << 2;
      const int base = ok ? nq * PN_LD + k : NB * PN_LD;
      const int step = ok ? PN_LD : 1;
      S[base] = r.x; S[base + step] = r.y; S[base + 2 * step] = r.z; S[base + 3 * step] = r.w;
    }
  };
  f32x4 acc[NTW];
#pragma unroll
  for (int b = 0; b < NTW; ++b) acc[b] = f32x4{0.f, 0.f, 0.f, 0.f};
  static_assert(BQ <= 3, "panel staging: at most 3 float4 per thread");
  float4 b0, b1, b2;
  float4 aC = load_a(0), aN;
  b0 = load_b(0, 0);
  if constexpr (BQ > 1) b1 = load_b(0, 1);
  if constexpr (BQ > 2) b2 = load_b(0, 2);
  store_b(sB[0], 0, b0);
  if constexpr (BQ > 1) store_b(sB[0], 1, b1);
  if constexpr (BQ > 2) store_b(sB[0], 2, b2);
  __syncthreads();
  for (int c = 0; c < nch; ++c) {
    const bool more = c + 1 < nch;
    if (more) {
      aN = load_a(c + 1);
      b0 = load_b(c + 1, 0);
      if constexpr (BQ > 1) b1 = load_b(c + 1, 1);
      if constexpr (BQ > 2) b2 = load_b(c + 1, 2);
    }
    const float* S = sB[c & 1];
    float4 bq[NTW];
#pragma unroll
    for (int b = 0; b < NTW; ++b)
      bq[b] = *reinterpret_cast<const float4*>(S + (16 * b + li) * PN_LD + 4 * lk);
#pragma unroll
    for (int b = 0; b < NTW; ++b) {
      acc[b] = mfma4(aC.x, bq[b].x, acc[b]);
      acc[b] = mfma4(aC.y, bq[b].y, acc[b]);
      acc[b] = mfma4(aC.z, bq[b].z, acc[b]);
      acc[b] = mfma4(aC.w, bq[b].w, acc[b]);
    }
    if (more) {
      float* S1 = sB[(c + 1) & 1];
      store_b(S1, 0, b0);
      if constexpr (BQ > 1) store_b(S1, 1, b1);
      if constexpr (BQ > 2) store_b(S1, 2, b2);
      aC = aN;
    }
    __syncthreads();
  }
#pragma unroll
  for (int b = 0; b < NTW; ++b) {
    const int n = n0 + 16 * b + li;
    if (n >= g.N) continue;
    float bias_n = 0.f;
    if constexpr (EPI == EPI_FWD) bias_n = g.bias ? g.bias[n] : 0.f;
#pragma unroll
    for (int i = 0; i < 4; ++i) {
      const int m = r0 + 4 * lk + i;
      if (m >= g.M) continue;
      float v = acc[b][i];
      if constexpr (EPI == EPI_FWD) {
        v += bias_n;
        if (g.act == ACT_RELU) v = v > 0.f ? v : 0.f;
        else if (g.act == ACT_TANH) v = tanhf(v);
      } else {
        if (g.mask) v = g.mask[(int64_t)m * g.ldm + n] > 0.f ? v : 0.f;
      }
      g.C[(int64_t)m * g.ldc + n] = v;
    }
  }
}

float* workspace_f32(int64_t nfloats);

static int smi_splitk_target() {
  static int t = 0;
  if (!t) {
    const char* e = getenv("SMI_SPLITK_TARGET");
    t = e ? atoi(e) : 512;
    if (t < 64) t = 64;
  }
  return t;
}

template <int EPI>
static void gemm_dispatch(const GemmArgs& g, dim3 grid, bool ak, bool bk, hipStream_t st) {
  if (ak && bk) hipLaunchKernelGGL((gemm_kernel<EPI, true, true>), grid, dim3(kWG), 0, st, g);
  else if (ak) hipLaunchKernelGGL((gemm_kernel<EPI, true, false>), grid, dim3(kWG), 0, st, g);
  else if (bk) hipLaunchKernelGGL((gemm_kernel<EPI, false, true>), grid, dim3(kWG), 0, st, g);
  else hipLaunchKernelGGL((gemm_kernel<EPI, false, false>), grid, dim3(kWG), 0, st, g);
}

static int use_dwd() {
  static int u = -1;
  if (u < 0) {
    const char* e = getenv("SMI_DWD");
    u = (e && e[0] == '0') ? 0 : 1;
  }
  return u;
}

template <int MT, int NT, int WV>
static void dwd_dispatch(const GemmArgs& g, dim3 grid, bool va, bool vb, hipStream_t st) {
  const size_t lds = (size_t)2 * MT * NT * 64 * sizeof(float4);
  const dim3 blk(64 * WV);
  if (va && vb) hipLaunchKernelGGL((gemm_dwd_kernel<MT, NT, true, true, WV>), grid, blk, lds, st, g);
  else if (va) hipLaunchKernelGGL((gemm_dwd_kernel<MT, NT, true, false, WV>), grid, blk, lds, st, g);
  else if (vb) hipLaunchKernelGGL((gemm_dwd_kernel<MT, NT, false, true, WV>), grid, blk, lds, st, g);
  else hipLaunchKernelGGL((gemm_dwd_kernel<MT, NT, false, false, WV>), grid, blk, lds, st, g);
}

static int dwd_waves() {
  static int w = 0;
  if (!w) {
    const char* e = getenv("SMI_DWD_WAVES");
    w = (e && atoi(e) == 8) ? 8 : 4;
  }
  return w;
}

static int splitk_reduce(const GemmArgs& g, int S, int epi, hipStream_t st, const char* what);

static int dwd_launch(GemmArgs g, hipStream_t st) {
  auto al16 = [](const float* p) { return (reinterpret_cast<uintptr_t>(p) & 15) == 0; };
  const int bdata = g.ones_col >= 0 ? g.ones_col : g.N;
  const int MT = g.M > 32 ? 4 : 1, NT = g.N > 64 ? 8 : 4;
  const bool va = MT == 4 && al16(g.A) && g.M % 4 == 0 && g.a_cs % 4 == 0;
  const bool vb = al16(g.B) && bdata >= 4 && bdata % 4 == 0 && g.b_rs % 4 == 0 &&
                  (!g.B2 || (al16(g.B2) && g.b2_rs % 4 == 0 && g.split_col % 4 == 0));
  const int gm = (g.M + 16 * MT - 1) / (16 * MT), gn = (g.N + 16 * NT - 1) / (16 * NT);
  const int tiles = gm * gn;
  static int target = 0;
  if (!target) {
    const char* e = getenv("SMI_DWD_TARGET");
    target = e ? atoi(e) : 256;
    if (target < 16) target = 16;
  }
  int S = (target + tiles - 1) / tiles;
  const int smax = (g.K + 32 * dwd_waves() - 1) / (32 * dwd_waves());
  if (S > smax) S = smax;
  const int64_t cap = smi_workspace_floats() / ((int64_t)g.M * g.N);
  if (S > cap) S = (int)cap;
  if (S < 1) S = 1;
  g.part = nullptr;
  g.kchunk = g.K;
  if (S > 1) {
    const int rs = 4 * dwd_waves() * DWD_P;
    g.kchunk = ((g.K + S - 1) / S + rs - 1) / rs * rs;
    S = (g.K + g.kchunk - 1) / g.kchunk;
  }
  if (S > 1) {
    g.part = workspace_f32((int64_t)S * g.M * g.N);
    if (!g.part) return set_error(SMI_E_ARG, "gemm: workspace unavailable for split-K");
  }
  const dim3 grid(gm, gn, S);
  const int kslot = ktime_begin(st);
  if (dwd_waves() == 8) {
    if (MT == 4 && NT == 8) dwd_dispatch<4, 8, 8>(g, grid, va, vb, st);
    else if (MT == 4) dwd_dispatch<4, 4, 8>(g, grid, va, vb, st);
    else if (NT == 8) dwd_dispatch<1, 8, 8>(g, grid, false, vb, st);
    else dwd_dispatch<1, 4, 8>(g, grid, false, vb, st);
  } else {
    if (MT == 4 && NT == 8) dwd_dispatch<4, 8, 4>(g, grid, va, vb, st);
    else if (MT == 4) dwd_dispatch<4, 4, 4>(g, grid, va, vb, st);
    else if (NT == 8) dwd_dispatch<1, 8, 4>(g, grid, false, vb, st);
    else dwd_dispatch<1, 4, 4>(g, grid, false, vb, st);
  }
  const int nreal = (g.ones_col >= 0 ? g.N - 1 : g.N) -
                    (g.B2 ? g.split_col - g.c1_real : 0);
  ktime_end(kslot, KT_GEMM_DW,
            2.0 * g.M * (double)nreal * g.K + (g.ones_col >= 0 ? (double)g.M * g.K : 0.0), st);
  const int rc = check_launch("gemm_dwd_kernel");
  if (rc || S == 1) return rc;
  return splitk_reduce(g, S, EPI_DW, st, "gemm_splitk_reduce_kernel<gemm_dwd_kernel>");
}

bool dw_group_takes(int M, int N) { return use_dwd() && M >= 1 && N >= 1 && M <= 512 && N <= 512; }

static thread_local DwGroup g_grp;
static thread_local bool g_grp_on = false;
static thread_local double g_grp_flops = 0.0;
static thread_local bool g_grp_missed = false;

int dw_group_begin() {
  g_grp_on = true;
  g_grp_missed = false;
  g_grp.n = 0;
  g_grp.x = DwEpilogue{};
  g_grp_flops = 0.0;
  return SMI_OK;
}

int dw_group_epilogue(const DwEpilogue& x) {
  if (!g_grp_on) return set_error(SMI_E_ARG, "dw group: no open group for the epilogue");
  g_grp.x = x;
  g_grp.x.on = 1;
  return SMI_OK;
}

static bool dw_group_add(const GemmArgs& g) {
  if (!g_grp_on) return false;
  if (g_grp.n >= kDwGroupMax) {
    g_grp_missed = true;
    return false;
  }
  auto al16 = [](const float* p) { return (reinterpret_cast<uintptr_t>(p) & 15) == 0; };
  const int bdata = g.ones_col >= 0 ? g.ones_col : g.N;
  const bool va = al16(g.A) && g.M >= 4 && g.M % 4 == 0 && g.a_cs % 4 == 0;
  const bool vb = al16(g.B) && bdata >= 4 && bdata % 4 == 0 && g.b_rs % 4 == 0 &&
                  (!g.B2 || (al16(g.B2) && g.b2_rs % 4 == 0 && g.split_col % 4 == 0));
  const int i = g_grp.n++;
  g_grp.g[i] = g;
  g_grp.vec[i] = (va ? 2 : 0) + (vb ? 1 : 0);
  const int nreal = (g.ones_col >= 0 ? g.N - 1 : g.N) - (g.B2 ? g.split_col - g.c1_real : 0);
  g_grp_flops += 2.0 * g.M * (double)nreal * g.K + (g.ones_col >= 0 ? (double)g.M * g.K : 0.0);
  return true;
}

static int dw_group_target(double work) {
  static int t = -1;
  if (t < 0) {
    const char* e = getenv("SMI_DWD_GROUP_TARGET");
    t = (e && e[0]) ? atoi(e) : 0;
    if (e && e[0] && t < 64) t = 64;
  }
  if (t > 0) return t;
  const double w = work / 256.0;
  return w >= 1536.0 ? 1536 : w <= 128.0 ? 128 : (int)w;
}

static int use_dwd_narrow() {
  static int u = -1;
  if (u < 0) {
    const char* e = getenv("SMI_DWD_NARROW");
    u = (e && e[0] == '0') ? 0 : 1;
  }
  return u;
}

static double dwd_narrow_cost() {
  static double c = -1.0;
  if (c < 0.0) {
    const char* e = getenv("SMI_DWD_NARROW_COST");
    c = (e && e[0]) ? atof(e) : 0.4;
    if (c <= 0.0 || c > 1.0) c = 0.4;
  }
  return c;
}

static int dwd_group_slots(size_t lds) {
  static int slots = 0;
  if (!slots) {
    slots = dwd_waves() == 8 ? resident_grid(gemm_dwd_group_kernel<8>, 512, lds)
                             : resident_grid(gemm_dwd_group_kernel<4>, 256, lds);
    if (slots < 1) slots = 256;
  }
  return slots;
}

static int red_u() {
  static const int u = [] { const char* e = getenv("SMI_RED_U"); return e && e[0] == '1' ? 1 : 4; }();
  return u;
}

static int dw_prepare(DwGroup& G, int wv, int slots, int64_t ws_off, int64_t& need,
                      int target_fixed = 0) {
  constexpr int MT = 4, NT = DWG_NT;
  const int rs = 4 * wv * DWD_P;
  auto al16 = [](const float* p) { return (reinterpret_cast<uintptr_t>(p) & 15) == 0; };
  {
    const int n0 = G.n;
    DwGroup E = G;
    int n = 0;
    for (int i = 0; i < n0; ++i) {
      const GemmArgs& g = G.g[i];
      const int tail = g.M % (16 * MT);
      const bool split = use_dwd_narrow() && tail > 0 && tail <= 16 && g.M > 16 * MT &&
                         g.a_rs == 1 && n + (n0 - i) + 1 <= kDwSplitMax;
      E.g[n] = g;
      E.vec[n] = G.vec[i];
      if (!split) { ++n; continue; }
      const int m0 = g.M - tail;
      E.g[n].M = m0;
      ++n;
      GemmArgs t = g;
      t.M = tail;
      t.A = g.A + m0;
      if (t.C) t.C = g.C + (int64_t)m0 * g.ldc;
      if (t.C2) t.C2 = g.C2 + (int64_t)m0 * g.ldc2;
      if (t.bias_out) t.bias_out = g.bias_out + m0;
      if (t.bias_out2) t.bias_out2 = g.bias_out2 + m0;
      const bool va = al16(t.A) && t.M >= 4 && t.M % 4 == 0 && t.a_cs % 4 == 0;
      E.g[n] = t;
      E.vec[n] = (va ? 2 : 0) + (G.vec[i] & 1);
      ++n;
    }
    E.n = n;
    G = E;
  }
  double cost[kDwGroupMax], work = 0.0, work_u = 0.0;
  int64_t tiles[kDwGroupMax];
  for (int i = 0; i < G.n; ++i) {
    const GemmArgs& g = G.g[i];
    const int tail = g.M % (16 * MT);
    G.narrow[i] = use_dwd_narrow() && tail > 0 && tail <= 16;
    G.gm[i] = (g.M + 16 * MT - 1) / (16 * MT);
    G.gn[i] = (g.N + 16 * NT - 1) / (16 * NT);
    tiles[i] = (int64_t)G.gm[i] * G.gn[i];
    cost[i] = G.narrow[i] ? ((G.gm[i] - 1) + dwd_narrow_cost()) / G.gm[i] : 1.0;
    work_u += (double)tiles[i] * g.K;
    work += (double)tiles[i] * g.K * cost[i];
  }
  int target = target_fixed > 0 ? target_fixed : dw_group_target(work_u);
  static const bool env_target = [] {
    const char* e = getenv("SMI_DWD_GROUP_TARGET");
    return e && e[0];
  }();
  const bool fixed_target = env_target || target_fixed > 0;
  if (!fixed_target && target >= slots) {
    static const double round_rows = [] {
      const char* e = getenv("SMI_DWD_ROUND_ROWS");
      const double v = (e && e[0]) ? atof(e) : 2048.0;
      return v >= 256.0 ? v : 2048.0;
    }();
    const int rounds = (int)std::max(1.0, std::ceil(work / (slots * round_rows)));
    target = slots * rounds;
  } else {
    for (int i = 0; i < G.n; ++i) cost[i] = 1.0;
    work = work_u;
  }
  const int64_t cap = smi_workspace_floats() - ws_off;
  double r0 = work / target;
  int64_t kcs[kDwGroupMax];
  const bool rounds_fit = !fixed_target && target >= slots;
  need = 0;
  for (int pass = 0; pass < 400; ++pass) {
    need = 0;
    int64_t wgs = 0;
    for (int i = 0; i < G.n; ++i) {
      const GemmArgs& g = G.g[i];
      int64_t S = (int64_t)(g.K * cost[i] / r0 + 0.5);
      if (S < 1) S = 1;
      int64_t kc = ((g.K + S - 1) / S + rs - 1) / rs * rs;
      if (kc < 2 * rs) kc = 2 * rs;
      if (kc >= g.K) kc = ((int64_t)g.K + rs - 1) / rs * rs;
      kcs[i] = kc;
      const int64_t s_i = (g.K + kc - 1) / kc;
      need += s_i * g.M * g.N;
      wgs += s_i * tiles[i];
    }
    if (need > cap) { r0 *= 2.0; continue; }
    if (rounds_fit && wgs > target && wgs <= 2 * target) { r0 *= 1.005; continue; }
    break;
  }
  float* base = workspace_f32(ws_off + need);
  if (!base) return set_error(SMI_E_ARG, "gemm: workspace too small for the grouped dW partials");
  base += ws_off;
  int64_t off = 0;
  G.wg0[0] = 0;
  G.rb0[0] = 0;
  for (int i = 0; i < G.n; ++i) {
    GemmArgs& g = G.g[i];
    g.kchunk = (int)kcs[i];
    G.S[i] = (int)((g.K + kcs[i] - 1) / kcs[i]);
    g.part = base + off;
    off += (int64_t)G.S[i] * g.M * g.N;
    G.wg0[i + 1] = G.wg0[i] + (int)(tiles[i] * G.S[i]);
    G.rb0[i + 1] = G.rb0[i] + (int)(((int64_t)g.M * g.N + 64 * red_u() - 1) / (64 * red_u()));
  }
  return SMI_OK;
}

constexpr int T16_MAXC = 8;
static bool use_t16() {
  static const bool on = [] { const char* e = getenv("SMI_GEMM_T16"); return !(e && e[0] == '0'); }();
  return on;
}

constexpr int DWT_DR = 8;
__global__ void __launch_bounds__(kWG)
gemm_dwt16_kernel(DwGroup G) {
  __shared__ f32x4 red[4][64];
  const int b = blockIdx.x;
  int gi = 0;
  while (gi + 1 < G.n && b >= G.wg0[gi + 1]) ++gi;
  const GemmArgs& g = G.g[gi];
  if (g.skip && g.skip[0] != 0) return;
  const int lane = threadIdx.x & 63, wave = threadIdx.x >> 6;
  const int i = lane & 15, q = lane >> 4;
  const int local = b - G.wg0[gi], gn16 = (g.N + 15) >> 4;
  const int m0 = (local / gn16) * 16, n0 = (local % gn16) * 16;
  const int mi = min(m0 + i, g.M - 1), ni = n0 + i;
  const int bdata = g.ones_col >= 0 ? g.ones_col : g.N;
  const float* Ar = g.A + (int64_t)mi * g.a_rs;
  const float* Bc = g.B;
  int64_t bs = g.b_rs;
  bool bz = false, bone = false;
  if (ni == g.ones_col) bone = true;
  else if (ni >= bdata || ni >= g.N) bz = true;
  else if (g.B2 && ni >= g.split_col) { Bc = g.B2 + (ni - g.split_col); bs = g.b2_rs; }
  else if (g.B2 && ni >= g.c1_real) bz = true;
  else Bc = g.B + (int64_t)ni * g.b_cs;
  const int nch = (g.K + 15) >> 4;
  const int nw = nch > wave ? (nch - wave + 3) >> 2 : 0;
  float av[DWT_DR][4], bv[DWT_DR][4];
  auto ld = [&](int j, int slot) {
    const int c = wave + 4 * j;
#pragma unroll
    for (int t = 0; t < 4; ++t) {
      const int k = 16 * c + 4 * q + t;
      const bool kv = j < nw && k < g.K;
      av[slot][t] = kv ? Ar[(int64_t)k * g.a_cs] : 0.f;
      bv[slot][t] = kv ? (bone ? 1.f : bz ? 0.f : Bc[(int64_t)k * bs]) : 0.f;
    }
  };
#pragma unroll
  for (int d = 0; d < DWT_DR; ++d) ld(d, d);
  f32x4 tot = {0.f, 0.f, 0.f, 0.f};
  for (int j0 = 0; j0 < nw; j0 += DWT_DR) {
    f32x4 acc[DWT_DR];
#pragma unroll
    for (int d = 0; d < DWT_DR; ++d) {
      acc[d] = f32x4{0.f, 0.f, 0.f, 0.f};
      if (j0 + d < nw) {
#pragma unroll
        for (int t = 0; t < 4; ++t) acc[d] = __builtin_amdgcn_mfma_f32_16x16x4f32(av[d][t], bv[d][t], acc[d], 0, 0, 0);
      }
      ld(j0 + d + DWT_DR, d);
    }
    tot += ((acc[0] + acc[1]) + (acc[2] + acc[3])) + ((acc[4] + acc[5]) + (acc[6] + acc[7]));
  }
  red[wave][lane] = tot;
  __syncthreads();
  if (wave != 0) return;
  const f32x4 sum = (red[0][lane] + red[1][lane]) + (red[2][lane] + red[3][lane]);
  if (ni >= g.N) return;
#pragma unroll
  for (int r = 0; r < 4; ++r) {
    const int m = m0 + 4 * q + r;
    if (m < g.M) dw_put(g, m, ni, sum[r]);
  }
}

static void dwt16_prefix(DwGroup& G) {
  G.wg0[0] = 0;
  for (int i = 0; i < G.n; ++i)
    G.wg0[i + 1] = G.wg0[i] + ((G.g[i].M + 15) / 16) * ((G.g[i].N + 15) / 16);
}

static thread_local DwGroup g_pre;
static thread_local bool g_pre_on = false;
static thread_local int64_t g_pre_need = 0;

constexpr size_t kDwdLds = (size_t)2 * 4 * DWG_NT * 64 * sizeof(float4);

int dw_group_flush(hipStream_t st) {
  g_grp_on = false;
  DwGroup& G = g_grp;
  const bool missed = g_grp_missed;
  g_grp_missed = false;
  const bool pre = g_pre_on;
  g_pre_on = false;
  struct Release { ~Release() { workspace_reserve(0); } } release_;
  if (G.x.on && G.x.sq && missed)
    return set_error(SMI_E_ARG, "dw group: a fused sum of squares needs every dW GEMM of the "
                                "bracket in the group (one ran outside it)");
  if (G.n == 0 && !pre) {
    if (!G.x.on) return SMI_OK;
    if (G.x.sq) return set_error(SMI_E_ARG, "dw group: fused sum of squares over an empty group");
    G.rb0[0] = 0;
    hipLaunchKernelGGL(gemm_group_reduce_kernel<1>, dim3(1), dim3(kWG), 0, st, G);
    return check_launch("gemm_group_reduce_kernel");
  }
  if (!pre && !G.x.on && use_t16()) {
    bool small = G.n > 0;
    for (int i = 0; i < G.n; ++i) small = small && G.g[i].K <= 4 * 16 * T16_MAXC;
    if (small) {
      dwt16_prefix(G);
      const int kslot = ktime_begin(st);
      hipLaunchKernelGGL(gemm_dwt16_kernel, dim3(G.wg0[G.n]), dim3(kWG), 0, st, G);
      ktime_end(kslot, KT_GEMM_DW, g_grp_flops, st);
      return check_launch("gemm_dwt16_kernel");
    }
  }
  int64_t need = 0;
  if (G.n > 0) {
    RC_CHECK(dw_prepare(G, dwd_waves(), dwd_group_slots(kDwdLds), 0, need));
    const int kslot = ktime_begin(st);
    if (dwd_waves() == 8)
      hipLaunchKernelGGL(gemm_dwd_group_kernel<8>, dim3(G.wg0[G.n]), dim3(512), kDwdLds, st, G);
    else
      hipLaunchKernelGGL(gemm_dwd_group_kernel<4>, dim3(G.wg0[G.n]), dim3(256), kDwdLds, st, G);
    ktime_end(kslot, KT_GEMM_DW, g_grp_flops, st);
    RC_CHECK(check_launch("gemm_dwd_group_kernel"));
  }
  DwGroup R = G;
  if (pre) {
    R = g_pre;
    R.x = G.x;
    if (R.n + G.n > kDwGroupMax) return set_error(SMI_E_ARG, "dw group: too many entries");
    for (int i = 0; i < G.n; ++i) {
      const int j = R.n + i;
      R.g[j] = G.g[i];
      R.S[j] = G.S[i];
      R.rb0[j + 1] = R.rb0[j] + (int)(((int64_t)G.g[i].M * G.g[i].N + 64 * red_u() - 1) / (64 * red_u()));
    }
    R.n += G.n;
    need += g_pre_need;
  }
  const int rslot = ktime_begin(st);
  if (red_u() == 4)
    hipLaunchKernelGGL(gemm_group_reduce_kernel<4>, dim3(R.rb0[R.n] + (R.x.on ? 1 : 0)), dim3(kWG), 0,
                       st, R);
  else
    hipLaunchKernelGGL(gemm_group_reduce_kernel<1>, dim3(R.rb0[R.n] + (R.x.on ? 1 : 0)), dim3(kWG), 0,
                       st, R);
  ktime_end(rslot, KT_GEMM_REDUCE, (double)need, st);
  return check_launch("gemm_group_reduce_kernel");
}

static bool use_bwd_dw() {
  static const bool on = [] { const char* e = getenv("SMI_BWD_DW"); return !(e && e[0] == '0'); }();
  return on;
}

int launch_lstm_bwd_dw(const float* dh, const float* gates, const float* cbuf, const float* w_hh,
                       int S, int B, int H, float* dgates, hipStream_t st, const int* skip) {
  const int br = lstm_bwd_q_form(B, H, w_hh);
  if (!use_bwd_dw() || !g_grp_on || g_pre_on || g_grp.n == 0 || br == 0 || S <= 0 || B <= 0)
    return SMI_E_NOFIT;
  int cus = 0, dev = 0;
  (void)hipGetDevice(&dev);
  if (hipDeviceGetAttribute(&cus, hipDeviceAttributeMultiprocessorCount, dev) != hipSuccess) cus = 256;
  if (cus - B < 32) return SMI_E_NOFIT;
  DwGroup Ga = g_grp;
  int64_t need = 0;
  RC_CHECK(dw_prepare(Ga, 8, cus - B, 0, need));
  static const bool excl = [] { const char* e = getenv("SMI_BWD_DW_EXCL"); return !(e && e[0] == '0'); }();
  size_t lds = excl ? std::max(kDwdLds, (size_t)84 * 1024) : kDwdLds;
  const size_t stg = (size_t)lstm_bwd_stage_floats(S, H) * 4;
  const bool stage = use_bwd_stage() && stg <= kBwdStageMax;
  if (stage) lds = std::max(lds, stg);
  LstmBwdArgs la{dh, gates, cbuf, w_hh, S, B, H, dgates, skip};
  const dim3 grid((unsigned)(B + Ga.wg0[Ga.n]));
  const int kslot = ktime_begin(st);
#define SMI_BD(BR_)                                                                          \
  do {                                                                                       \
    if (stage) {                                                                             \
      allow_lds(lstm_bwd_dw_kernel<BR_, true>, lds);                                         \
      hipLaunchKernelGGL((lstm_bwd_dw_kernel<BR_, true>), grid, dim3(kVT), lds, st, la, Ga); \
    } else {                                                                                 \
      allow_lds(lstm_bwd_dw_kernel<BR_, false>, lds);                                        \
      hipLaunchKernelGGL((lstm_bwd_dw_kernel<BR_, false>), grid, dim3(kVT), lds, st, la, Ga);\
    }                                                                                        \
  } while (0)
  if (br == 16) SMI_BD(16);
  else if (br == 25) SMI_BD(25);
  else SMI_BD(32);
#undef SMI_BD
  ktime_end(kslot, KT_LSTM_BWD, 8.0 * B * H * (double)H * (S - 1), st);
  RC_CHECK(check_launch("lstm_bwd_dw_kernel"));
  g_pre = Ga;
  g_pre_on = true;
  g_pre_need = need;
  workspace_reserve(need);
  g_grp.n = 0;
  g_grp_flops = 0.0;
  return SMI_OK;
}

static int use_panel() {
  static int u = -1;
  if (u < 0) {
    const char* e = getenv("SMI_PANEL");
    u = (e && e[0] == '0') ? 0 : 1;
  }
  return u;
}

template <int EPI>
static const char* panel_dispatch(const GemmArgs& g, dim3 grid, int ntw, hipStream_t st) {
#define SMI_PN(C)                                                                      \
  hipLaunchKernelGGL((gemm_panel_kernel<EPI, C>), grid, dim3(kWG), 0, st, g);          \
  return EPI == EPI_FWD ? "gemm_panel_kernel<fwd," #C ">" : "gemm_panel_kernel<dx," #C ">"
  switch (ntw) {
    case 1: SMI_PN(1);
    case 2: SMI_PN(2);
    case 4: SMI_PN(4);
    case 5: SMI_PN(5);
    case 7: SMI_PN(7);
    default: SMI_PN(10);
  }
#undef SMI_PN
}

static bool panel_ok(int epi, const GemmArgs& g) {
  auto al16 = [](const void* p) { return (reinterpret_cast<uintptr_t>(p) & 15) == 0; };
  static const int panel_min_rows = [] {
    const char* e = getenv("SMI_PANEL_MIN_ROWS");
    return e ? atoi(e) : 4096;
  }();
  if (!use_panel() || g.M < panel_min_rows || g.N > 640 || g.K > 1024 || g.K < 1) return false;
  if (g.a_cs != 1 || g.a_rs % 4 || g.K % 4 || !al16(g.A) || !al16(g.B)) return false;
  if (epi == EPI_FWD) return g.b_rs == 1 && g.b_cs % 4 == 0;
  static const int dx_min = [] {
    const char* e = getenv("SMI_PANEL_DX_MIN");
    return e ? atoi(e) : 96;
  }();
  if (epi == EPI_DX)
    return g.b_cs == 1 && g.b_rs % 4 == 0 && g.N % 4 == 0 && g.N >= dx_min;
  return false;
}

static int panel_launch(int epi, const GemmArgs& g, hipStream_t st) {
  static const int cand[6] = {1, 2, 4, 5, 7, 10};
  const int t16 = (g.N + 15) / 16;
  int best = 10;
  double bcost = 1e30;
  for (int c : cand) {
    const int groups = (t16 + c - 1) / c;
    const double cost = groups * c + 0.3 * groups;
    if (cost < bcost) { bcost = cost; best = c; }
  }
  const dim3 grid((g.M + 63) / 64, (g.N + 16 * best - 1) / (16 * best), 1);
  const int kslot = ktime_begin(st);
  const char* form = epi == EPI_FWD ? panel_dispatch<EPI_FWD>(g, grid, best, st)
                                    : panel_dispatch<EPI_DX>(g, grid, best, st);
  ktime_end(kslot, epi == EPI_FWD ? KT_GEMM_FWD : KT_GEMM_DX, 2.0 * g.M * (double)g.N * g.K, st);
  return check_launch(form);
}

template <int KK, bool V4, bool A4 = false>
__global__ void __launch_bounds__(kWG)
dx_smallk_kernel(GemmArgs g) {
  if (g.skip && g.skip[0] != 0) return;
  constexpr int RW = 4;
  const int nq = (g.N + 3) >> 2;
  const int64_t idx = (int64_t)blockIdx.x * kWG + threadIdx.x;
  if (idx >= (int64_t)((g.M + RW - 1) / RW) * nq) return;
  const int mg = (int)(idx / nq), n0 = (int)(idx - (int64_t)mg * nq) * 4;
  float w[KK][4];
#pragma unroll
  for (int k = 0; k < KK; ++k) {
    const float* wr = g.B + (int64_t)min(k, g.K - 1) * g.b_rs;
    if constexpr (V4) {
      const float4 x = *reinterpret_cast<const float4*>(wr + n0);
      w[k][0] = x.x; w[k][1] = x.y; w[k][2] = x.z; w[k][3] = x.w;
    } else {
#pragma unroll
      for (int t = 0; t < 4; ++t) w[k][t] = wr[min(n0 + t, g.N - 1)];
    }
  }
#pragma unroll
  for (int r = 0; r < RW; ++r) {
    const int m = mg * RW + r;
    if (m >= g.M) break;
    const float* arow = g.A + (int64_t)m * g.a_rs;
    float av[KK];
    if (KK % 4 == 0 && A4) {
#pragma unroll
      for (int q = 0; q < KK / 4; ++q) {
        const float4 x = reinterpret_cast<const float4*>(arow)[q];
        av[4 * q] = x.x; av[4 * q + 1] = x.y; av[4 * q + 2] = x.z; av[4 * q + 3] = x.w;
      }
    } else {
#pragma unroll
      for (int k = 0; k < KK; ++k) av[k] = k < g.K ? arow[k] : 0.f;
    }
    float v[4] = {0.f, 0.f, 0.f, 0.f};
#pragma unroll
    for (int k = 0; k < KK; ++k) {
      if (k >= g.K) break;
#pragma unroll
      for (int t = 0; t < 4; ++t) v[t] = fmaf(av[k], w[k][t], v[t]);
    }
    const float* mrow = g.mask ? g.mask + (int64_t)m * g.ldm + n0 : nullptr;
    float* crow = g.C + (int64_t)m * g.ldc + n0;
    if constexpr (V4) {
      if (mrow) {
        const float4 mk = *reinterpret_cast<const float4*>(mrow);
        v[0] = mk.x > 0.f ? v[0] : 0.f; v[1] = mk.y > 0.f ? v[1] : 0.f;
        v[2] = mk.z > 0.f ? v[2] : 0.f; v[3] = mk.w > 0.f ? v[3] : 0.f;
      }
      *reinterpret_cast<float4*>(crow) = float4{v[0], v[1], v[2], v[3]};
    } else {
#pragma unroll
      for (int t = 0; t < 4; ++t) {
        if (n0 + t >= g.N) break;
        crow[t] = (mrow && !(mrow[t] > 0.f)) ? 0.f : v[t];
      }
    }
  }
}

static int use_dx_smallk() {
  static int u = -1;
  if (u < 0) {
    const char* e = getenv("SMI_DX_SMALLK");
    u = (e && e[0] == '0') ? 0 : 1;
  }
  return u;
}

static int dx_smallk_launch(const GemmArgs& g, hipStream_t st) {
  auto al16 = [](const void* p) { return (reinterpret_cast<uintptr_t>(p) & 15) == 0; };
  const bool v4 = g.N % 4 == 0 && g.ldc % 4 == 0 && al16(g.C) && g.b_rs % 4 == 0 && al16(g.B) &&
                  (!g.mask || (g.ldm % 4 == 0 && al16(g.mask)));
  const int64_t n = (int64_t)((g.M + 3) / 4) * ((g.N + 3) / 4);
  const dim3 grid((unsigned)((n + kWG - 1) / kWG));
  const int kslot = ktime_begin(st);
  const char* form;
#define SMI_DXS(KK)                                                                        \
  do {                                                                                     \
    if (v4) hipLaunchKernelGGL((dx_smallk_kernel<KK, true>), grid, dim3(kWG), 0, st, g);   \
    else hipLaunchKernelGGL((dx_smallk_kernel<KK, false>), grid, dim3(kWG), 0, st, g);     \
    form = v4 ? "dx_smallk_kernel<" #KK ",v4>" : "dx_smallk_kernel<" #KK ">";              \
  } while (0)
  const bool a4 = (g.K == 4 || g.K == 8) && g.a_rs % 4 == 0 && al16(g.A);
  if (g.K == 1) SMI_DXS(1);
  else if (g.K <= 2) SMI_DXS(2);
  else if (g.K == 8 && a4 && v4) {
    hipLaunchKernelGGL((dx_smallk_kernel<8, true, true>), grid, dim3(kWG), 0, st, g);
    form = "dx_smallk_kernel<8,v4,a4>";
  }
  else if (g.K <= 4) SMI_DXS(4);
  else SMI_DXS(8);
#undef SMI_DXS
  ktime_end(kslot, KT_GEMM_DX, 2.0 * g.M * (double)g.N * g.K, st);
  return check_launch(form);
}

template <int EPI>
__global__ void __launch_bounds__(kWG)
gemm_t16_kernel(GemmArgs g) {
  if (g.skip && g.skip[0] != 0) return;
  __shared__ f32x4 red[4][64];
  const int lane = threadIdx.x & 63, wave = threadIdx.x >> 6;
  const int i = lane & 15, q = lane >> 4;
  const int m0 = blockIdx.x * 16, n0 = blockIdx.y * 16;
  const int ra = min(m0 + i, g.M - 1), cb = min(n0 + i, g.N - 1);
  const float* Ar = g.A + (int64_t)ra * g.a_rs;
  const float* Bc = g.B + (int64_t)cb * g.b_cs;
  const int nch = (g.K + 15) >> 4;
  const bool a4 = g.avec && g.a_cs == 1, b4 = g.bvec && g.b_rs == 1;
  float av[T16_MAXC][4], bv[T16_MAXC][4];
#pragma unroll
  for (int j = 0; j < T16_MAXC; ++j) {
    const int c = wave + 4 * j;
    const int k0 = 16 * c + 4 * q;
    if (c >= nch) break;
    if (a4 && k0 + 3 < g.K) {
      const float4 x = *reinterpret_cast<const float4*>(Ar + k0);
      av[j][0] = x.x; av[j][1] = x.y; av[j][2] = x.z; av[j][3] = x.w;
    } else {
#pragma unroll
      for (int t = 0; t < 4; ++t) av[j][t] = k0 + t < g.K ? Ar[(int64_t)(k0 + t) * g.a_cs] : 0.f;
    }
    if (b4 && k0 + 3 < g.K) {
      const float4 x = *reinterpret_cast<const float4*>(Bc + k0);
      bv[j][0] = x.x; bv[j][1] = x.y; bv[j][2] = x.z; bv[j][3] = x.w;
    } else {
#pragma unroll
      for (int t = 0; t < 4; ++t) bv[j][t] = k0 + t < g.K ? Bc[(int64_t)(k0 + t) * g.b_rs] : 0.f;
    }
  }
  f32x4 acc = {0.f, 0.f, 0.f, 0.f};
#pragma unroll
  for (int j = 0; j < T16_MAXC; ++j) {
    if (wave + 4 * j >= nch) break;
#pragma unroll
    for (int t = 0; t < 4; ++t) acc = __builtin_amdgcn_mfma_f32_16x16x4f32(av[j][t], bv[j][t], acc, 0, 0, 0);
  }
  red[wave][lane] = acc;
  __syncthreads();
  if (EPI == EPI_FWD && wave == 1 && blockIdx.y == 0 && g.xsrc) {
    for (int e = lane; e < 16 * g.xcols; e += 64) {
      const int r = e / g.xcols, j = e - r * g.xcols;
      if (m0 + r < g.M) g.C[(int64_t)(m0 + r) * g.ldc + g.N + j] = g.xsrc[(int64_t)(m0 + r) * g.xlds + j];
    }
  }
  if (wave != 0) return;
  const f32x4 sum = (red[0][lane] + red[1][lane]) + (red[2][lane] + red[3][lane]);
  const int n = n0 + i;
  if (n >= g.N) return;
#pragma unroll
  for (int r = 0; r < 4; ++r) {
    const int m = m0 + 4 * q + r;
    if (m >= g.M) continue;
    float v = sum[r];
    if constexpr (EPI == EPI_FWD) {
      if (g.bias) v += g.bias[n];
      if (g.act == ACT_RELU) v = v > 0.f ? v : 0.f;
      else if (g.act == ACT_TANH) v = tanhf(v);
    } else {
      if (g.mask && !(g.mask[(int64_t)m * g.ldm + n] > 0.f)) v = 0.f;
    }
    g.C[(int64_t)m * g.ldc + n] = v;
  }
}


static int gemm_launch(int epi, GemmArgs g, hipStream_t st) {
  if (g.M <= 0 || g.N <= 0) return SMI_OK;
  g.part = nullptr;
  if (epi == EPI_DX && use_dx_smallk() && g.K >= 1 && g.K <= 8 && g.a_cs == 1 && g.b_cs == 1)
    return dx_smallk_launch(g, st);
  if (epi != EPI_DW && !g.xsrc && panel_ok(epi, g)) return panel_launch(epi, g, st);
  if (epi == EPI_DW) {
    const bool grp_ok = use_dwd() && g.a_rs == 1 && g.b_cs == 1 && g.K >= 1 &&
                        (g.ones_col >= 0 ? g.ones_col : g.N) >= 1 && g.M <= 512 && g.N <= 512;
    if (grp_ok && dw_group_add(g)) return SMI_OK;
    if (g_grp_on) g_grp_missed = true;
    if (grp_ok) return dwd_launch(g, st);
  }
  const bool ak = g.a_cs == 1;
  const bool bk = g.b_rs == 1;
  auto al16 = [](const float* p) { return (reinterpret_cast<uintptr_t>(p) & 15) == 0; };
  g.avec = al16(g.A) && (ak ? (g.K % 4 == 0 && g.a_rs % 4 == 0) : (g.a_rs == 1 && g.M % 4 == 0 && g.a_cs % 4 == 0));
  const int bdata = g.ones_col >= 0 ? g.ones_col : g.N;
  g.bvec = al16(g.B) && (bk ? (g.K % 4 == 0 && g.b_cs % 4 == 0) : (g.b_cs == 1 && bdata % 4 == 0 && g.b_rs % 4 == 0));
  const int breal = g.ones_col >= 0 ? g.ones_col : g.N;
  const bool dw128 = epi == EPI_DW && !ak && !bk && g.a_rs == 1 && g.b_cs == 1 &&
                     al16(g.A) && al16(g.B) && g.M % 4 == 0 && breal % 4 == 0 &&
                     g.a_cs % 4 == 0 && g.b_rs % 4 == 0 && g.M >= 96 && g.N >= 96 &&
                     g.K >= 1024;
  const int TM = dw128 ? D2_T : GBM, TN = dw128 ? D2_T : GBN;
  const int gm = (g.M + TM - 1) / TM, gn = (g.N + TN - 1) / TN;
  int S = 1;
  g.part = nullptr;
  g.kchunk = g.K > 0 ? g.K : 1;
  static const int fwd_split_min = [] {
    const char* e = getenv("SMI_FWD_SPLITK_MIN");
    return e ? atoi(e) : 4 * GBK;
  }();
  const bool split_fwd = (epi == EPI_FWD || epi == EPI_DX) && gm * gn < 256 &&
                         g.K >= fwd_split_min;
  if ((epi == EPI_FWD || epi == EPI_DX) && gm * gn < 256 && use_t16() && g.M <= 4096 &&
      g.K <= 4 * 16 * T16_MAXC) {
    const dim3 grid16((g.M + 15) / 16, (g.N + 15) / 16);
    const int kslot = ktime_begin(st);
    if (epi == EPI_FWD) hipLaunchKernelGGL(gemm_t16_kernel<EPI_FWD>, grid16, dim3(kWG), 0, st, g);
    else hipLaunchKernelGGL(gemm_t16_kernel<EPI_DX>, grid16, dim3(kWG), 0, st, g);
    ktime_end(kslot, epi == EPI_FWD ? KT_GEMM_FWD : KT_GEMM_DX, 2.0 * g.M * (double)g.N * g.K, st);
    return check_launch(epi == EPI_FWD ? "gemm_t16_kernel<fwd>" : "gemm_t16_kernel<dx>");
  }
  if ((epi == EPI_DW && g.K > 4 * GBK) || split_fwd) {
    const int tiles = gm * gn;
    S = (smi_splitk_target() + tiles - 1) / tiles;
    const int smax = (g.K + 4 * GBK - 1) / (4 * GBK);
    if (S > smax) S = smax;
    const int64_t cap = smi_workspace_floats() / ((int64_t)g.M * g.N);
    if (S > cap) S = (int)cap;
    if (S < 1) S = 1;
    if (dw128 && (g.K + S - 1) / S > 512) S = (g.K + 511) / 512;
    if (S > cap) S = (int)cap;
    if (S < 1) S = 1;
    if (S > 1) {
      g.kchunk = ((g.K + S - 1) / S + 31) / 32 * 32;
      S = (g.K + g.kchunk - 1) / g.kchunk;
      g.part = workspace_f32((int64_t)S * g.M * g.N);
      if (!g.part) return set_error(SMI_E_ARG, "gemm: workspace unavailable for split-K");
    }
  }
  const dim3 grid(gm, gn, S);
  const int kslot = ktime_begin(st);
  if (dw128) hipLaunchKernelGGL(gemm_dw128_kernel, grid, dim3(kWG), 0, st, g);
  else if (epi == EPI_FWD) gemm_dispatch<EPI_FWD>(g, grid, ak, bk, st);
  else if (epi == EPI_DX) gemm_dispatch<EPI_DX>(g, grid, ak, bk, st);
  else gemm_dispatch<EPI_DW>(g, grid, ak, bk, st);
  const int nreal = g.ones_col >= 0 ? g.N - 1 : g.N;
  ktime_end(kslot, epi == EPI_FWD ? KT_GEMM_FWD : epi == EPI_DX ? KT_GEMM_DX : KT_GEMM_DW,
            2.0 * g.M * (double)nreal * g.K + (g.ones_col >= 0 ? (double)g.M * g.K : 0.0), st);
  int rc = check_launch(dw128 ? "gemm_dw128_kernel" : epi == EPI_FWD ? "gemm_kernel<fwd>"
                        : epi == EPI_DX ? "gemm_kernel<dx>" : "gemm_kernel<dw>");
  if (rc || S == 1) return rc;
  return splitk_reduce(g, S, epi, st,
                       dw128 ? "gemm_splitk_reduce_kernel<gemm_dw128_kernel>"
                       : epi == EPI_FWD ? "gemm_splitk_reduce_kernel<gemm_kernel<fwd>>"
                       : epi == EPI_DX ? "gemm_splitk_reduce_kernel<gemm_kernel<dx>>"
                                       : "gemm_splitk_reduce_kernel<gemm_kernel<dw>>");
}

static int splitk_reduce(const GemmArgs& g, int S, int epi, hipStream_t st, const char* what) {
  const int rslot = ktime_begin(st);
  const int64_t MN = (int64_t)g.M * g.N;
  const int rg = (int)((MN + 63) / 64);
  const bool fwd = epi == EPI_FWD;
  hipLaunchKernelGGL(gemm_splitk_reduce_kernel, dim3(rg), dim3(kWG), 0, st, g.part, S, g,
                     fwd ? g.bias : nullptr, fwd ? g.act : ACT_NONE,
                     epi == EPI_DX ? g.mask : nullptr);
  ktime_end(rslot, KT_GEMM_REDUCE, (double)S * MN, st);
  return check_launch(what);
}

int launch_slab_reduce(const float* part, int S, int64_t n, float* out, hipStream_t st,
                       const int* skip) {
  if (n < 1 || S < 1) return SMI_OK;
  const int rg = (int)((n + 63) / 64);
  GemmArgs g{};
  g.M = 1; g.N = (int)n; g.C = out; g.ldc = n; g.ones_col = -1; g.skip = skip;
  hipLaunchKernelGGL(gemm_splitk_reduce_kernel, dim3(rg), dim3(kWG), 0, st, part, S, g, nullptr,
                     ACT_NONE, nullptr);
  return check_launch("gemm_splitk_reduce_kernel");
}

int launch_linear_fwd(const float* X, int64_t ldx, int M, int K, const float* W, int64_t ldw,
                      const float* b, int N, int act, float* Y, int64_t ldy, hipStream_t st,
                      const int* skip) {
  if (K >= 1 && K <= 64 && N >= 32 && N <= 512 && M >= 2048)
    return launch_smallk_fwd(X, ldx, M, K, W, ldw, b, N, act, Y, ldy, st, skip);
  GemmArgs g{};
  g.M = M; g.N = N; g.K = K;
  g.A = X; g.a_rs = ldx; g.a_cs = 1;
  g.B = W; g.b_rs = 1; g.b_cs = ldw;
  g.C = Y; g.ldc = ldy; g.bias = b; g.act = act; g.ones_col = -1; g.skip = skip;
  return gemm_launch(EPI_FWD, g, st);
}

int launch_copy_cols(const float* src, int64_t lds, int64_t rows, int cols, float* dst,
                     int64_t ldd, hipStream_t st);
int launch_linear_fwd_cat(const float* X, int64_t ldx, int M, int K, const float* W, int64_t ldw,
                          const float* b, int N, int act, float* Y, int64_t ldy, const float* S,
                          int64_t lds, int xcols, hipStream_t st) {
  const int gm = (M + GBM - 1) / GBM, gn = (N + GBN - 1) / GBN;
  const bool t16 = !(K >= 1 && K <= 64 && N >= 32 && N <= 512 && M >= 2048) && use_t16() &&
                   gm * gn < 256 && M <= 4096 && K <= 4 * 16 * T16_MAXC && M > 0;
  if (!t16) {
    RC_CHECK(launch_linear_fwd(X, ldx, M, K, W, ldw, b, N, act, Y, ldy, st));
    return launch_copy_cols(S, lds, M, xcols, Y + N, ldy, st);
  }
  GemmArgs g{};
  g.M = M; g.N = N; g.K = K;
  g.A = X; g.a_rs = ldx; g.a_cs = 1;
  g.B = W; g.b_rs = 1; g.b_cs = ldw;
  g.C = Y; g.ldc = ldy; g.bias = b; g.act = act; g.ones_col = -1;
  g.xsrc = S; g.xlds = lds; g.xcols = xcols;
  return gemm_launch(EPI_FWD, g, st);
}

int launch_linear_bwd_dx(const float* dY, int64_t ldg, int M, int N, const float* W, int64_t ldw,
                         int K, const float* mask, int64_t ldm, float* dX, int64_t lddx,
                         hipStream_t st, const int* skip) {
  GemmArgs g{};
  g.M = M; g.N = K; g.K = N;
  g.A = dY; g.a_rs = ldg; g.a_cs = 1;
  g.B = W; g.b_rs = ldw; g.b_cs = 1;
  g.C = dX; g.ldc = lddx; g.mask = mask; g.ldm = ldm; g.ones_col = -1; g.skip = skip;
  return gemm_launch(EPI_DX, g, st);
}

int launch_linear_bwd_dw2(const float* dY, int64_t ldg, int M, int N, const float* X1,
                          int64_t ldx1, int K1, const float* X2, int64_t ldx2, int K2,
                          float* dW1, int64_t ld1, float* dW2, int64_t ld2, float* db1,
                          float* db2, hipStream_t st, const int* skip) {
  const int K1p = (int)ldx1;
  if (K1p < K1 || K1p % 4) return set_error(SMI_E_ARG, "bwd_dw2: ldx1 must be a multiple of 4 >= K1");
  GemmArgs g{};
  g.M = N; g.N = K1p + K2 + 1; g.K = M;
  g.A = dY; g.a_rs = 1; g.a_cs = ldg;
  g.B = X1; g.b_rs = ldx1; g.b_cs = 1;
  g.B2 = X2; g.b2_rs = ldx2; g.split_col = K1p; g.c1_real = K1;
  g.C = dW1; g.ldc = ld1; g.C2 = dW2; g.ldc2 = ld2;
  g.ones_col = K1p + K2; g.bias_out = db1; g.bias_out2 = db2; g.skip = skip;
  if (!(g.a_rs == 1 && g.b_cs == 1 && use_dwd() && g.M <= 512 && g.N <= 512))
    return set_error(SMI_E_ARG, "bwd_dw2: shape not supported");
  if (dw_group_add(g)) return SMI_OK;
  if (g_grp_on) g_grp_missed = true;
  return dwd_launch(g, st);
}

int launch_linear_bwd_dw(const float* dY, int64_t ldg, int M, int N, const float* X, int64_t ldx,
                         int K, float* dW, int64_t lddw, float* db, int accumulate,
                         hipStream_t st, const int* skip) {
  GemmArgs g{};
  g.M = N; g.N = db ? K + 1 : K; g.K = M;
  g.A = dY; g.a_rs = 1; g.a_cs = ldg;
  g.B = X; g.b_rs = ldx; g.b_cs = 1;
  g.C = dW; g.ldc = lddw; g.accumulate = accumulate; g.skip = skip;
  g.ones_col = db ? K : -1;
  g.bias_out = db;
  return gemm_launch(EPI_DW, g, st);
}

}
```

Before: 3.744 million env-steps/s.

## Split grouped dW GEMMs into planned sub-tile entries with narrow tile classes

```diff
diff --git a/include/surreal_mi.h b/include/surreal_mi.h
--- a/include/surreal_mi.h
+++ b/include/surreal_mi.h
@@ -295,6 +295,8 @@
                                float* db, int accumulate, void* stream);
 int smi_dw_group_begin(void);
 int smi_dw_group_flush(void* stream);
+int smi_diag_dw_plan(const int* gemms, int ng, int waves, int slots, int64_t cap_floats,
+                     int max_ent, int64_t* out, int64_t* tot);
 
 int smi_mse_grad(const float* q, int64_t q_stride, const float* y, int64_t n, float* dq,
                  float* loss, void* stream);
diff --git a/surreal_amd/_lib.py b/surreal_amd/_lib.py
--- a/surreal_amd/_lib.py
+++ b/surreal_amd/_lib.py
@@ -127,6 +127,7 @@
     'smi_reward_filter_commit': (c_int, [P, P, P, P, P]),
     'smi_dw_group_begin': (c_int, []),
     'smi_dw_group_flush': (c_int, [P]),
+    'smi_diag_dw_plan': (c_int, [P, c_int, c_int, c_int, c_i64, c_int, P, P]),
     'smi_layernorm_forward': (c_int, [P, c_i64, c_i64, c_int, P, P, c_f32, P, c_i64, P, P, P]),
     'smi_layernorm_backward': (c_int, [P, c_i64, P, c_i64, P, P, P, c_i64, c_int, c_int, P, c_i64,
                                        P, P, P]),
diff --git a/surreal_amd/csrc/linear_kernels.hip b/surreal_amd/csrc/linear_kernels.hip
--- a/surreal_amd/csrc/linear_kernels.hip
+++ b/surreal_amd/csrc/linear_kernels.hip
@@ -579,6 +579,37 @@
 constexpr int DWD_P = SMI_DWD_P;
 
 
+typedef float dwd_v2 __attribute__((ext_vector_type(2), aligned(4)));
+typedef float dwd_v3 __attribute__((ext_vector_type(3), aligned(4)));
+template <int W, bool GLOBAL>
+__device__ __forceinline__ float4 dwd_ldw(const float* p) {
+#define SMI_LDW(T_) (GLOBAL ? *(const __attribute__((address_space(1))) T_*)p : *(const T_*)p)
+  if constexpr (W == 4) { const f32x4 x = SMI_LDW(f32x4); return float4{x[0], x[1], x[2], x[3]}; }
+  else if constexpr (W == 3) { const dwd_v3 x = SMI_LDW(dwd_v3); return float4{x[0], x[1], x[2], 0.f}; }
+  else if constexpr (W == 2) { const dwd_v2 x = SMI_LDW(dwd_v2); return float4{x[0], x[1], 0.f, 0.f}; }
+  else return float4{SMI_LDW(float), 0.f, 0.f, 0.f};
+#undef SMI_LDW
+}
+
+template <int W>
+__device__ __forceinline__ int dwd_fit_col(int c0, int lim, int li, int j) {
+  const int cb = c0 + W * li;
+  const int c = min(cb, lim - W) + j;
+  return c >= cb ? c : -1;
+}
+
+struct DwEnt {
+  float* part;
+  int gi;
+  int m0, n0, M, N;
+  int kchunk, S;
+  int gm, gn;
+  int cls;
+};
+__host__ __device__ constexpr int dw_cls(int mt, int nt, bool va, bool vb) {
+  return mt | (nt << 3) | ((mt == 4 && va) << 7) | ((nt >= 4 && vb) << 8);
+}
+
 template <int MT, int NT, bool VA, bool VB, int NB = NT>
 __device__ __forceinline__ void dwd_load(const GemmArgs& g, int r, int ke, int m0, int n0, int bdata,
                                          float (&av)[MT], float (&bv)[NT]) {
@@ -595,9 +626,24 @@
     const int c = min(m0 + 4 * li, g.M - 4);
     const float4 x = *reinterpret_cast<const float4*>(Ar + c);
     av[0] = x.x; av[1] = x.y; av[2] = x.z; av[3] = x.w;
+  } else if constexpr (MT == 2 || MT == 3) {
+    const float4 x = dwd_ldw<MT, false>(Ar + min(m0 + MT * li, g.M - MT));
+    av[0] = x.x; av[1] = x.y;
+    if constexpr (MT == 3) av[2] = x.z;
   } else {
 #pragma unroll
     for (int t = 0; t < MT; ++t) av[t] = Ar[min(m0 + MT * li + t, g.M - 1)];
+  }
+  if constexpr (NT < 4) {
+    const int cb = n0 + NT * li;
+    const int c = min(cb, bdata - NT);
+    const float* src = cb < bdata ? (c >= split ? Br2 : Br) + c
+                                  : (g.ones_col >= 0 && cb < bdata + NT ? one : g_dwd_zero);
+    const float4 x = dwd_ldw<NT, false>(src);
+    bv[0] = x.x;
+    if constexpr (NT >= 2) bv[1] = x.y;
+    if constexpr (NT == 3) bv[2] = x.z;
+    return;
   }
 #pragma unroll
   for (int h = 0; h < NB / 4; ++h) {
@@ -626,41 +672,39 @@
 template <int MT, int NT, int NB, int RS>
 __device__ __forceinline__ void dwd_main_fast(const GemmArgs& g, int rw, int nsteps, int m0, int n0,
                                               int bdata, f32x4 (&acc)[MT][NT]) {
-  static_assert(MT == 4 || MT == 1, "fast dW loop: 4 m sub-tiles (float4 A) or 1 (scalar A)");
-  constexpr int NH = NB / 4;
+  static_assert(NB == NT || (NT == 8 && NB == 4), "fast dW loop: whole tiles or the lower half of 8");
+  constexpr int GW = NT < 4 ? NT : 4;
+  constexpr int NH = NB / GW;
   const int li = threadIdx.x & 15;
-  const float* pa = g.A + (int64_t)rw * g.a_cs + (MT == 4 ? min(m0 + 4 * li, g.M - 4)
-                                                          : min(m0 + li, g.M - 1));
+  const float* pa = g.A + (int64_t)rw * g.a_cs + min(m0 + MT * li, g.M - MT);
   const int64_t sa = (int64_t)RS * g.a_cs;
   const float* pb[NH];
   int64_t sb[NH];
 #pragma unroll
   for (int h = 0; h < NH; ++h) {
-    const int cb = n0 + 64 * h + 4 * li;
+    const int cb = n0 + 64 * h + GW * li;
     if (cb < bdata) {
-      if (g.B2 && cb >= g.split_col) {
-        pb[h] = g.B2 + (int64_t)rw * g.b2_rs + (cb - g.split_col);
+      const int c = NT < 4 ? min(cb, bdata - NT) : cb;
+      if (g.B2 && c >= g.split_col) {
+        pb[h] = g.B2 + (int64_t)rw * g.b2_rs + (c - g.split_col);
         sb[h] = (int64_t)RS * g.b2_rs;
       } else {
-        pb[h] = g.B + (int64_t)rw * g.b_rs + cb;
+        pb[h] = g.B + (int64_t)rw * g.b_rs + c;
         sb[h] = (int64_t)RS * g.b_rs;
       }
     } else {
-      pb[h] = cb == g.ones_col ? g_dwd_one : g_dwd_zero;
+      const bool ones = NT < 4 ? g.ones_col >= 0 && cb < bdata + NT : cb == g.ones_col;
+      pb[h] = ones ? g_dwd_one : g_dwd_zero;
       sb[h] = 0;
     }
   }
   float4 av[DWD_P], bv[DWD_P][NH];
-  using gf4 = const __attribute__((address_space(1))) f32x4;
-  using gf1 = const __attribute__((address_space(1))) float;
-  auto f4 = [](const f32x4 x) { return float4{x[0], x[1], x[2], x[3]}; };
   auto load = [&](int p) {
-    if constexpr (MT == 4) av[p] = f4(*(gf4*)pa);
-    else av[p].x = *(gf1*)pa;
+    av[p] = dwd_ldw<MT, true>(pa);
     pa += sa;
 #pragma unroll
     for (int h = 0; h < NH; ++h) {
-      bv[p][h] = f4(*(gf4*)pb[h]);
+      bv[p][h] = dwd_ldw<GW, true>(pb[h]);
       pb[h] += sb[h];
     }
   };
@@ -685,10 +729,13 @@
     load(p);
     __builtin_amdgcn_sched_barrier(0);
   }
+  constexpr bool kRestart = MT == 1;
   f32x4 tot[MT][NT];
-  if constexpr (MT == 1) {
-#pragma unroll
-    for (int b = 0; b < NT; ++b) tot[0][b] = f32x4{0.f, 0.f, 0.f, 0.f};
+  if constexpr (kRestart) {
+#pragma unroll
+    for (int a = 0; a < MT; ++a)
+#pragma unroll
+      for (int b = 0; b < NT; ++b) tot[a][b] = f32x4{0.f, 0.f, 0.f, 0.f};
   }
   for (int s0 = DWD_P; s0 < nsteps; s0 += DWD_P) {
 #pragma unroll
@@ -697,29 +744,35 @@
       if constexpr (SMI_DWD_DIAG != 1) load(p);
       __builtin_amdgcn_sched_barrier(0);
     }
-    if constexpr (MT == 1) {
-#pragma unroll
-      for (int b = 0; b < NB; ++b) {
-        tot[0][b] += acc[0][b];
-        acc[0][b] = f32x4{0.f, 0.f, 0.f, 0.f};
-      }
+    if constexpr (kRestart) {
+#pragma unroll
+      for (int a = 0; a < MT; ++a)
+#pragma unroll
+        for (int b = 0; b < NB; ++b) {
+          tot[a][b] += acc[a][b];
+          acc[a][b] = f32x4{0.f, 0.f, 0.f, 0.f};
+        }
     }
   }
 #pragma unroll
   for (int p = 0; p < DWD_P; ++p) step(p);
-  if constexpr (MT == 1) {
-#pragma unroll
-    for (int b = 0; b < NB; ++b) acc[0][b] = tot[0][b] + acc[0][b];
+  if constexpr (kRestart) {
+#pragma unroll
+    for (int a = 0; a < MT; ++a)
+#pragma unroll
+      for (int b = 0; b < NB; ++b) acc[a][b] = tot[a][b] + acc[a][b];
   }
 }
 
 template <int MT, int NT, bool VA, bool VB, int WV>
-__device__ __forceinline__ void dwd_tile(const GemmArgs& g, const TileIdx ti, float4* dwd_red) {
+__device__ __forceinline__ void dwd_tile(const GemmArgs& g, const DwEnt& e, const TileIdx ti,
+                                         float4* dwd_red) {
   const int lane = threadIdx.x & 63, wave = threadIdx.x >> 6;
   const int li = lane & 15, lk = lane >> 4;
-  const int m0 = ti.mt * 16 * MT, n0 = ti.nt * 16 * NT;
-  const int kb = ti.z * g.kchunk;
-  const int ke = min(g.K, kb + g.kchunk);
+  const int m0 = e.m0 + ti.mt * 16 * MT, n0 = e.n0 + ti.nt * 16 * NT;
+  const int mend = e.m0 + e.M, nend = e.n0 + e.N;
+  const int kb = ti.z * e.kchunk;
+  const int ke = min(g.K, kb + e.kchunk);
   constexpr int RS = 4 * WV;
   const int nsteps = (ke - kb + RS - 1) / RS;
   const int bdata = g.ones_col >= 0 ? g.ones_col : g.N;
@@ -747,12 +800,12 @@
       }
     }
   };
-  constexpr bool kFast = VB && ((VA && MT == 4) || MT == 1);
+  constexpr bool kFast = (VB || NT < 4) && (VA || MT < 4);
   bool fast = false;
   if constexpr (kFast)
     fast = use_dwd_fast() && nsteps >= DWD_P && nsteps % DWD_P == 0 && kb + nsteps * RS <= ke;
   constexpr int NBH = NT > 4 ? 4 : NT;
-  if (NT == 8 && n0 + 64 >= g.N) {
+  if (NT == 8 && n0 + 64 >= nend) {
     if constexpr (kFast) {
       if (fast) dwd_main_fast<MT, NT, NBH, RS>(g, rw, nsteps, m0, n0, bdata, acc);
       else mainloop(std::integral_constant<int, NBH>{});
@@ -796,19 +849,35 @@
     }
   }
   if (wave != 0) return;
-  const bool vec_part = g.part && (g.N & 3) == 0;
+  auto out = [&](int m, int n, float v) {
+    if (e.part) e.part[((int64_t)ti.z * e.M + (m - e.m0)) * e.N + (n - e.n0)] = v;
+    else dw_put(g, m, n, v);
+  };
+  const bool vec_part = e.part && (e.N & 3) == 0;
 #pragma unroll
   for (int a = 0; a < MT; ++a)
 #pragma unroll
     for (int i = 0; i < 4; ++i) {
-      const int m = m0 + MT * (lk * 4 + i) + a;
-      if (m >= g.M) continue;
+      int m = m0 + MT * (lk * 4 + i) + a;
+      if constexpr (MT == 2 || MT == 3) m = dwd_fit_col<MT>(m0, g.M, lk * 4 + i, a);
+      if (m < 0 || m >= mend) continue;
+      if constexpr (NT < 4) {
+        const int cb = n0 + NT * li;
+#pragma unroll
+        for (int t = 0; t < NT; ++t) {
+          int n = cb < bdata ? dwd_fit_col<NT>(n0, bdata, li, t)
+                             : (t == 0 && g.ones_col >= 0 && cb < bdata + NT ? g.ones_col : -1);
+          if (n < 0 || n >= nend) continue;
+          out(m, n, acc[a][t][i]);
+        }
+        continue;
+      }
 #pragma unroll
       for (int h = 0; h < NT / 4; ++h) {
         const int nb = n0 + 64 * h + 4 * li;
         if (vec_part) {
-          if (nb < g.N)
-            *reinterpret_cast<float4*>(g.part + ((int64_t)ti.z * g.M + m) * g.N + nb) =
+          if (nb < nend)
+            *reinterpret_cast<float4*>(e.part + ((int64_t)ti.z * e.M + (m - e.m0)) * e.N + (nb - e.n0)) =
                 float4{acc[a][4 * h][i], acc[a][4 * h + 1][i], acc[a][4 * h + 2][i],
                        acc[a][4 * h + 3][i]};
           continue;
@@ -816,10 +885,8 @@
 #pragma unroll
         for (int t = 0; t < 4; ++t) {
           const int n = nb + t;
-          if (n >= g.N) continue;
-          const float v = acc[a][4 * h + t][i];
-          if (g.part) g.part[((int64_t)ti.z * g.M + m) * g.N + n] = v;
-          else dw_put(g, m, n, v);
+          if (n >= nend) continue;
+          out(m, n, acc[a][4 * h + t][i]);
         }
       }
     }
@@ -830,21 +897,24 @@
 gemm_dwd_kernel(GemmArgs g) {
   if (g.skip && g.skip[0] != 0) return;
   extern __shared__ float4 dwd_red[];
-  dwd_tile<MT, NT, VA, VB, WV>(g, gemm_tile_index(), dwd_red);
-}
-
-constexpr int kDwGroupMax = 8;
-constexpr int kDwSplitMax = 6;
+  DwEnt e{};
+  e.part = g.part; e.M = g.M; e.N = g.N; e.kchunk = g.kchunk;
+  dwd_tile<MT, NT, VA, VB, WV>(g, e, gemm_tile_index(), dwd_red);
+}
+
+constexpr int kDwGemmMax = 8;
+constexpr int kDwGroupMax = 16;
+constexpr int kDwSplitMax = 16;
 struct DwGroup {
   DwEpilogue x;
-  GemmArgs g[kDwGroupMax];
+  GemmArgs g[kDwGemmMax];
+  DwEnt e[kDwGroupMax];
   int wg0[kDwGroupMax + 1];
   int rb0[kDwGroupMax + 1];
-  int gm[kDwGroupMax], gn[kDwGroupMax], S[kDwGroupMax];
-  int vec[kDwGroupMax];
-  int narrow[kDwGroupMax];
-  int n;
+  int vec[kDwGemmMax];
+  int ng, n;
 };
+static_assert(sizeof(DwGroup) + 128 <= 4096, "DwGroup must fit the kernel-argument segment");
 
 #ifndef SMI_DWG_NT
 #define SMI_DWG_NT 4
@@ -865,35 +935,49 @@
 
 template <int WV>
 __device__ __forceinline__ void dwd_group_run(const DwGroup& G, int orig, int nwg, float4* dwd_red,
-                                              int& gi, int& rows) {
+                                              int& ei, int& rows) {
   int w = orig;
   if (nwg > 8) {
     const int x = orig & 7, q = nwg >> 3, r = nwg & 7;
     w = (x < r ? x * (q + 1) : r * (q + 1) + (x - r) * q) + (orig >> 3);
   }
-  gi = 0;
-  while (gi + 1 < G.n && w >= G.wg0[gi + 1]) ++gi;
-  const GemmArgs& g = G.g[gi];
+  ei = 0;
+  while (ei + 1 < G.n && w >= G.wg0[ei + 1]) ++ei;
+  const DwEnt e = G.e[ei];
+  const GemmArgs g = G.g[e.gi];
   if (g.skip && g.skip[0] != 0) return;
-  const int local = w - G.wg0[gi], gn = G.gn[gi], gm = G.gm[gi];
+  const int local = w - G.wg0[ei];
   TileIdx ti;
-  ti.nt = local % gn;
-  ti.mt = (local / gn) % gm;
-  ti.z = local / (gn * gm);
-  rows = (min(g.K, (ti.z + 1) * g.kchunk) - ti.z * g.kchunk) |
-         ((G.narrow[gi] && ti.mt == gm - 1) << 16) | (G.vec[gi] << 17);
-  if (G.narrow[gi] && ti.mt == gm - 1) {
-    ti.mt *= 4;
-    if (G.vec[gi] & 1) dwd_tile<1, DWG_NT, false, true, WV>(g, ti, dwd_red);
-    else dwd_tile<1, DWG_NT, false, false, WV>(g, ti, dwd_red);
-    return;
-  }
-  switch (G.vec[gi]) {
-    case 3: dwd_tile<4, DWG_NT, true, true, WV>(g, ti, dwd_red); break;
-    case 2: dwd_tile<4, DWG_NT, true, false, WV>(g, ti, dwd_red); break;
-    case 1: dwd_tile<4, DWG_NT, false, true, WV>(g, ti, dwd_red); break;
-    default: dwd_tile<4, DWG_NT, false, false, WV>(g, ti, dwd_red); break;
-  }
+  ti.nt = local % e.gn;
+  ti.mt = (local / e.gn) % e.gm;
+  ti.z = local / (e.gn * e.gm);
+  rows = (min(g.K, (ti.z + 1) * e.kchunk) - ti.z * e.kchunk) | (e.cls << 16);
+#define SMI_DWT(MT_, NT_, VA_, VB_) \
+  case dw_cls(MT_, NT_, VA_, VB_): dwd_tile<MT_, NT_, VA_, VB_, WV>(g, e, ti, dwd_red); break;
+#define SMI_DWT3(NT_, VB_) SMI_DWT(1, NT_, false, VB_) SMI_DWT(2, NT_, false, VB_) SMI_DWT(3, NT_, false, VB_)
+  switch (e.cls) {
+    SMI_DWT(4, DWG_NT, true, true) SMI_DWT(4, DWG_NT, true, false)
+    SMI_DWT(4, DWG_NT, false, true) SMI_DWT(4, DWG_NT, false, false)
+    SMI_DWT(1, DWG_NT, false, true) SMI_DWT(1, DWG_NT, false, false)
+    default: break;
+  }
+#if SMI_DWG_NT == 4
+#define SMI_DWT_FIT 1
+#else
+#define SMI_DWT_FIT 0
+#endif
+  if constexpr (SMI_DWT_FIT && WV == 4) {
+    switch (e.cls) {
+      SMI_DWT(2, DWG_NT, false, true) SMI_DWT(3, DWG_NT, false, true)
+      SMI_DWT(2, DWG_NT, false, false) SMI_DWT(3, DWG_NT, false, false)
+      SMI_DWT(4, 1, true, false) SMI_DWT(4, 2, true, false) SMI_DWT(4, 3, true, false)
+      SMI_DWT(4, 1, false, false) SMI_DWT(4, 2, false, false) SMI_DWT(4, 3, false, false)
+      SMI_DWT3(1, false) SMI_DWT3(2, false) SMI_DWT3(3, false)
+      default: break;
+    }
+  }
+#undef SMI_DWT3
+#undef SMI_DWT
 }
 
 template <int WV>
@@ -1063,17 +1147,18 @@
     return;
   }
   const int b = (int)blockIdx.x - ep;
-  int gi = 0;
-  while (gi + 1 < G.n && b >= G.rb0[gi + 1]) ++gi;
-  const GemmArgs& g = G.g[gi];
+  int ei = 0;
+  while (ei + 1 < G.n && b >= G.rb0[ei + 1]) ++ei;
+  const DwEnt& en = G.e[ei];
+  const GemmArgs& g = G.g[en.gi];
   if (g.skip && g.skip[0] != 0) return;
-  const int S = G.S[gi];
-  const int64_t MN = (int64_t)g.M * g.N;
+  const int S = en.S;
+  const int64_t MN = (int64_t)en.M * en.N;
   const int el = threadIdx.x & 63, zl = threadIdx.x >> 6;
-  const int64_t eb = (int64_t)(b - G.rb0[gi]) * 64 * U;
+  const int64_t eb = (int64_t)(b - G.rb0[ei]) * 64 * U;
   const float* p[U];
 #pragma unroll
-  for (int u = 0; u < U; ++u) p[u] = g.part + min(eb + el + 64 * u, MN - 1);
+  for (int u = 0; u < U; ++u) p[u] = en.part + min(eb + el + 64 * u, MN - 1);
   float r[U];
   red_slabs<U>(p, MN, S, zl, r);
 #pragma unroll
@@ -1084,8 +1169,8 @@
     const int64_t e = eb + i;
     if (e < MN) {
       const float v = (red[0][i] + red[1][i]) + (red[2][i] + red[3][i]);
-      const int m = (int)(e / g.N), n = (int)(e - (int64_t)m * g.N);
-      q += dw_put(g, m, n, v);
+      const int m = (int)(e / en.N), n = (int)(e - (int64_t)m * en.N);
+      q += dw_put(g, en.m0 + m, en.n0 + n, v);
     }
   }
   if (!G.x.sq) return;
@@ -1321,7 +1406,7 @@
 int dw_group_begin() {
   g_grp_on = true;
   g_grp_missed = false;
-  g_grp.n = 0;
+  g_grp.ng = g_grp.n = 0;
   g_grp.x = DwEpilogue{};
   g_grp_flops = 0.0;
   return SMI_OK;
@@ -1336,7 +1421,7 @@
 
 static bool dw_group_add(const GemmArgs& g) {
   if (!g_grp_on) return false;
-  if (g_grp.n >= kDwGroupMax) {
+  if (g_grp.ng >= kDwGemmMax) {
     g_grp_missed = true;
     return false;
   }
@@ -1345,9 +1430,10 @@
   const bool va = al16(g.A) && g.M >= 4 && g.M % 4 == 0 && g.a_cs % 4 == 0;
   const bool vb = al16(g.B) && bdata >= 4 && bdata % 4 == 0 && g.b_rs % 4 == 0 &&
                   (!g.B2 || (al16(g.B2) && g.b2_rs % 4 == 0 && g.split_col % 4 == 0));
-  const int i = g_grp.n++;
+  const int i = g_grp.ng++;
   g_grp.g[i] = g;
-  g_grp.vec[i] = (va ? 2 : 0) + (vb ? 1 : 0);
+  g_grp.vec[i] = (va ? 2 : 0) + (vb ? 1 : 0) + (al16(g.A) ? 4 : 0) +
+                 (al16(g.B) && (!g.B2 || al16(g.B2)) ? 8 : 0);
   const int nreal = (g.ones_col >= 0 ? g.N - 1 : g.N) - (g.B2 ? g.split_col - g.c1_real : 0);
   g_grp_flops += 2.0 * g.M * (double)nreal * g.K + (g.ones_col >= 0 ? (double)g.M * g.K : 0.0);
   return true;
@@ -1390,6 +1476,13 @@
     slots = dwd_waves() == 8 ? resident_grid(gemm_dwd_group_kernel<8>, 512, lds)
                              : resident_grid(gemm_dwd_group_kernel<4>, 256, lds);
     if (slots < 1) slots = 256;
+    if (dwd_waves() == 4) {
+      int dev = 0, cus = 0;
+      (void)hipGetDevice(&dev);
+      if (hipDeviceGetAttribute(&cus, hipDeviceAttributeMultiprocessorCount, dev) == hipSuccess &&
+          cus > 0 && slots > cus * SMI_DWG_OCC)
+        slots = cus * SMI_DWG_OCC;
+    }
   }
   return slots;
 }
@@ -1399,53 +1492,98 @@
   return u;
 }
 
-static int dw_prepare(DwGroup& G, int wv, int slots, int64_t ws_off, int64_t& need,
-                      int target_fixed = 0) {
-  constexpr int MT = 4, NT = DWG_NT;
+struct DwPlanGemm {
+  int M, N, K;
+  int vec;
+  int ones;
+  int split_col;
+};
+struct DwPlanEnt {
+  int gi, m0, n0, M, N, mt, nt, cls, gm, gn, kchunk, S;
+  int64_t part_off;
+};
+struct DwPlan {
+  DwPlanEnt e[kDwSplitMax];
+  int wg0[kDwSplitMax + 1], rb0[kDwSplitMax + 1];
+  int n;
+  int64_t need;
+};
+
+static int dw_plan_rects(const DwPlanGemm& p, int gi, int fit, DwPlanEnt* out) {
+  const bool va = (p.vec & 2) != 0, vb = (p.vec & 1) != 0;
+  auto ent = [&](int m0, int n0, int M, int N, int mt, int nt) {
+    DwPlanEnt e{};
+    e.gi = gi; e.m0 = m0; e.n0 = n0; e.M = M; e.N = N; e.mt = mt; e.nt = nt;
+    e.cls = dw_cls(mt, nt, va, vb);
+    e.gm = (M + 16 * mt - 1) / (16 * mt);
+    e.gn = (N + 16 * nt - 1) / (16 * nt);
+    return e;
+  };
+  const int Mf = p.M / 64 * 64, Me = p.M - Mf, Nf = p.N / 64 * 64, Ne = p.N - Nf;
+  if (fit == 1 && Me >= 1 && Me <= 16) {
+    int k = 0;
+    if (Mf) out[k++] = ent(0, 0, Mf, p.N, 4, DWG_NT);
+    out[k++] = ent(Mf, 0, Me, p.N, 1, DWG_NT);
+    return k;
+  }
+  if (fit < 2) {
+    out[0] = ent(0, 0, p.M, p.N, 4, DWG_NT);
+    return 1;
+  }
+  int mte = (Me + 15) / 16, nte = 0;
+  if ((mte == 2 || mte == 3) && !(p.vec & 4)) mte = 4;
+  if (Ne > 0) {
+    const int R = Ne - (p.ones ? 1 : 0);
+    nte = p.ones ? std::max(1, (R + 14) / 15) : (R + 15) / 16;
+    if (nte > 4) nte = 4;
+    if (p.split_col >= 0 && nte > 1 && Nf < p.split_col) nte = 4;
+    if ((nte == 2 || nte == 3) && !(p.vec & 8)) nte = 4;
+    if (mte == 1 && !vb) nte = 4;
+  }
+  int n = 0;
+  if (Mf && Nf) out[n++] = ent(0, 0, Mf, Nf, 4, 4);
+  if (Me && Nf) out[n++] = ent(Mf, 0, Me, Nf, mte, 4);
+  if (Mf && Ne) out[n++] = ent(0, Nf, Mf, Ne, 4, nte);
+  if (Me && Ne) out[n++] = ent(Mf, Nf, Me, Ne, mte, nte);
+  return n;
+}
+
+static int dw_fit_level(int wv) {
+  if (!use_dwd_narrow()) return 0;
+  return wv == 4 && DWG_NT == 4 ? 2 : 1;
+}
+
+static int dw_plan(const DwPlanGemm* gemms, int ng, int wv, int slots, int64_t cap, int max_ent,
+                   int target_fixed, DwPlan& P) {
+  constexpr int kBandMax = 6;
+  constexpr int NTF = DWG_NT;
   const int rs = 4 * wv * DWD_P;
-  auto al16 = [](const float* p) { return (reinterpret_cast<uintptr_t>(p) & 15) == 0; };
-  {
-    const int n0 = G.n;
-    DwGroup E = G;
-    int n = 0;
-    for (int i = 0; i < n0; ++i) {
-      const GemmArgs& g = G.g[i];
-      const int tail = g.M % (16 * MT);
-      const bool split = use_dwd_narrow() && tail > 0 && tail <= 16 && g.M > 16 * MT &&
-                         g.a_rs == 1 && n + (n0 - i) + 1 <= kDwSplitMax;
-      E.g[n] = g;
-      E.vec[n] = G.vec[i];
-      if (!split) { ++n; continue; }
-      const int m0 = g.M - tail;
-      E.g[n].M = m0;
-      ++n;
-      GemmArgs t = g;
-      t.M = tail;
-      t.A = g.A + m0;
-      if (t.C) t.C = g.C + (int64_t)m0 * g.ldc;
-      if (t.C2) t.C2 = g.C2 + (int64_t)m0 * g.ldc2;
-      if (t.bias_out) t.bias_out = g.bias_out + m0;
-      if (t.bias_out2) t.bias_out2 = g.bias_out2 + m0;
-      const bool va = al16(t.A) && t.M >= 4 && t.M % 4 == 0 && t.a_cs % 4 == 0;
-      E.g[n] = t;
-      E.vec[n] = (va ? 2 : 0) + (G.vec[i] & 1);
-      ++n;
-    }
-    E.n = n;
-    G = E;
-  }
-  double cost[kDwGroupMax], work = 0.0, work_u = 0.0;
-  int64_t tiles[kDwGroupMax];
-  for (int i = 0; i < G.n; ++i) {
-    const GemmArgs& g = G.g[i];
-    const int tail = g.M % (16 * MT);
-    G.narrow[i] = use_dwd_narrow() && tail > 0 && tail <= 16;
-    G.gm[i] = (g.M + 16 * MT - 1) / (16 * MT);
-    G.gn[i] = (g.N + 16 * NT - 1) / (16 * NT);
-    tiles[i] = (int64_t)G.gm[i] * G.gn[i];
-    cost[i] = G.narrow[i] ? ((G.gm[i] - 1) + dwd_narrow_cost()) / G.gm[i] : 1.0;
-    work_u += (double)tiles[i] * g.K;
-    work += (double)tiles[i] * g.K * cost[i];
+  if (max_ent > kDwSplitMax) max_ent = kDwSplitMax;
+  struct Band { int gi, m0, M; int64_t tiles; double cost; int64_t kc; };
+  Band band[2 * kDwGemmMax];
+  int nb = 0, tail_band[kDwGemmMax];
+  int first_band[kDwGemmMax];
+  double work = 0.0, work_u = 0.0;
+  for (int i = 0; i < ng; ++i) {
+    const DwPlanGemm& g = gemms[i];
+    const int tail = g.M % 64, gn = (g.N + 16 * NTF - 1) / (16 * NTF);
+    const bool narrow = use_dwd_narrow() && tail > 0 && tail <= 16;
+    const bool cut = narrow && g.M > 64 && nb + (ng - i) + 1 <= kBandMax;
+    first_band[i] = nb;
+    tail_band[i] = -1;
+    if (cut) {
+      band[nb++] = Band{i, 0, g.M - tail, (int64_t)(g.M / 64) * gn, 1.0, 0};
+      tail_band[i] = nb;
+      band[nb++] = Band{i, g.M - tail, tail, gn, dwd_narrow_cost(), 0};
+    } else {
+      const int gm = (g.M + 63) / 64;
+      band[nb++] = Band{i, 0, g.M, (int64_t)gm * gn,
+                        narrow ? ((gm - 1) + dwd_narrow_cost()) / gm : 1.0, 0};
+    }
+  }
+  for (int b = 0; b < nb; ++b) {
+    work_u += (double)band[b].tiles * gemms[band[b].gi].K;
+    work += (double)band[b].tiles * gemms[band[b].gi].K * band[b].cost;
   }
   int target = target_fixed > 0 ? target_fixed : dw_group_target(work_u);
   static const bool env_target = [] {
@@ -1462,48 +1600,108 @@
     const int rounds = (int)std::max(1.0, std::ceil(work / (slots * round_rows)));
     target = slots * rounds;
   } else {
-    for (int i = 0; i < G.n; ++i) cost[i] = 1.0;
+    for (int b = 0; b < nb; ++b) band[b].cost = 1.0;
     work = work_u;
   }
-  const int64_t cap = smi_workspace_floats() - ws_off;
   double r0 = work / target;
-  int64_t kcs[kDwGroupMax];
   const bool rounds_fit = !fixed_target && target >= slots;
-  need = 0;
   for (int pass = 0; pass < 400; ++pass) {
-    need = 0;
-    int64_t wgs = 0;
-    for (int i = 0; i < G.n; ++i) {
-      const GemmArgs& g = G.g[i];
-      int64_t S = (int64_t)(g.K * cost[i] / r0 + 0.5);
+    int64_t need = 0, wgs = 0;
+    for (int b = 0; b < nb; ++b) {
+      const DwPlanGemm& g = gemms[band[b].gi];
+      int64_t S = (int64_t)(g.K * band[b].cost / r0 + 0.5);
       if (S < 1) S = 1;
       int64_t kc = ((g.K + S - 1) / S + rs - 1) / rs * rs;
       if (kc < 2 * rs) kc = 2 * rs;
       if (kc >= g.K) kc = ((int64_t)g.K + rs - 1) / rs * rs;
-      kcs[i] = kc;
-      const int64_t s_i = (g.K + kc - 1) / kc;
-      need += s_i * g.M * g.N;
-      wgs += s_i * tiles[i];
+      band[b].kc = kc;
+      const int64_t s_b = (g.K + kc - 1) / kc;
+      need += s_b * band[b].M * g.N;
+      wgs += s_b * band[b].tiles;
     }
     if (need > cap) { r0 *= 2.0; continue; }
     if (rounds_fit && wgs > target && wgs <= 2 * target) { r0 *= 1.005; continue; }
     break;
   }
+  P.n = 0;
+  for (int i = 0; i < ng; ++i) {
+    DwPlanEnt r[4];
+    int k = 0;
+    for (int fit = dw_fit_level(wv); fit >= 0; --fit) {
+      k = dw_plan_rects(gemms[i], i, fit, r);
+      if (P.n + k + (ng - 1 - i) <= max_ent) break;
+    }
+    if (k == 0 || P.n + k > max_ent) return -1;
+    for (int j = 0; j < k; ++j) {
+      const int b = tail_band[i] >= 0 && r[j].m0 >= band[tail_band[i]].m0 ? tail_band[i] : first_band[i];
+      r[j].kchunk = (int)band[b].kc;
+      r[j].S = (int)((gemms[i].K + band[b].kc - 1) / band[b].kc);
+      P.e[P.n++] = r[j];
+    }
+  }
+  int64_t off = 0;
+  P.wg0[0] = 0;
+  P.rb0[0] = 0;
+  for (int i = 0; i < P.n; ++i) {
+    DwPlanEnt& e = P.e[i];
+    e.part_off = off;
+    off += ((int64_t)e.S * e.M * e.N + 3) / 4 * 4;
+    P.wg0[i + 1] = P.wg0[i] + e.gm * e.gn * e.S;
+    P.rb0[i + 1] = P.rb0[i] + (int)(((int64_t)e.M * e.N + 64 * red_u() - 1) / (64 * red_u()));
+  }
+  if (off > cap) return -1;
+  P.need = off;
+  return 0;
+}
+
+extern "C" int smi_diag_dw_plan(const int* gemms, int ng, int waves, int slots, int64_t cap_floats,
+                                int max_ent, int64_t* out, int64_t* tot) {
+  if (!gemms || !out || !tot || ng < 1 || ng > kDwGemmMax || (waves != 4 && waves != 8) ||
+      slots < 1 || max_ent < 1)
+    return set_error(SMI_E_ARG, "smi_diag_dw_plan: bad arguments");
+  DwPlanGemm pg[kDwGemmMax];
+  for (int i = 0; i < ng; ++i) {
+    pg[i] = DwPlanGemm{gemms[6 * i], gemms[6 * i + 1], gemms[6 * i + 2], gemms[6 * i + 3],
+                       gemms[6 * i + 4], gemms[6 * i + 5]};
+    if (pg[i].M < 1 || pg[i].N < 1 || pg[i].K < 1 || pg[i].M > 512 || pg[i].N > 512)
+      return set_error(SMI_E_ARG, "smi_diag_dw_plan: GEMM outside the grouped kernel's range");
+  }
+  DwPlan P;
+  if (dw_plan(pg, ng, waves, slots, cap_floats, max_ent, 0, P))
+    return set_error(SMI_E_ARG, "smi_diag_dw_plan: the partials do not fit");
+  for (int i = 0; i < P.n; ++i) {
+    const DwPlanEnt& e = P.e[i];
+    const int64_t row[12] = {e.gi, e.m0, e.n0, e.M, e.N, e.mt, e.nt, e.kchunk, e.S,
+                             P.wg0[i], P.rb0[i], e.part_off};
+    for (int j = 0; j < 12; ++j) out[12 * i + j] = row[j];
+  }
+  tot[0] = P.wg0[P.n]; tot[1] = P.rb0[P.n]; tot[2] = P.need; tot[3] = 4 * waves * DWD_P;
+  return P.n;
+}
+
+static int dw_prepare(DwGroup& G, int wv, int slots, int64_t ws_off, int64_t& need, int max_ent,
+                      int target_fixed = 0) {
+  DwPlanGemm pg[kDwGemmMax];
+  for (int i = 0; i < G.ng; ++i) {
+    const GemmArgs& g = G.g[i];
+    pg[i] = DwPlanGemm{g.M, g.N, g.K, G.vec[i], g.ones_col >= 0 ? 1 : 0, g.B2 ? g.split_col : -1};
+  }
+  DwPlan P;
+  if (dw_plan(pg, G.ng, wv, slots, smi_workspace_floats() - ws_off, max_ent, target_fixed, P))
+    return set_error(SMI_E_ARG, "gemm: workspace too small for the grouped dW partials");
+  need = P.need;
   float* base = workspace_f32(ws_off + need);
   if (!base) return set_error(SMI_E_ARG, "gemm: workspace too small for the grouped dW partials");
   base += ws_off;
-  int64_t off = 0;
-  G.wg0[0] = 0;
-  G.rb0[0] = 0;
-  for (int i = 0; i < G.n; ++i) {
-    GemmArgs& g = G.g[i];
-    g.kchunk = (int)kcs[i];
-    G.S[i] = (int)((g.K + kcs[i] - 1) / kcs[i]);
-    g.part = base + off;
-    off += (int64_t)G.S[i] * g.M * g.N;
-    G.wg0[i + 1] = G.wg0[i] + (int)(tiles[i] * G.S[i]);
-    G.rb0[i + 1] = G.rb0[i] + (int)(((int64_t)g.M * g.N + 64 * red_u() - 1) / (64 * red_u()));
-  }
+  G.n = P.n;
+  for (int i = 0; i < P.n; ++i) {
+    const DwPlanEnt& p = P.e[i];
+    DwEnt& e = G.e[i];
+    e.part = base + p.part_off;
+    e.gi = p.gi; e.m0 = p.m0; e.n0 = p.n0; e.M = p.M; e.N = p.N;
+    e.kchunk = p.kchunk; e.S = p.S; e.gm = p.gm; e.gn = p.gn; e.cls = p.cls;
+  }
+  for (int i = 0; i <= P.n; ++i) { G.wg0[i] = P.wg0[i]; G.rb0[i] = P.rb0[i]; }
   return SMI_OK;
 }
 
@@ -1519,7 +1717,7 @@
   __shared__ f32x4 red[4][64];
   const int b = blockIdx.x;
   int gi = 0;
-  while (gi + 1 < G.n && b >= G.wg0[gi + 1]) ++gi;
+  while (gi + 1 < G.ng && b >= G.wg0[gi + 1]) ++gi;
   const GemmArgs& g = G.g[gi];
   if (g.skip && g.skip[0] != 0) return;
   const int lane = threadIdx.x & 63, wave = threadIdx.x >> 6;
@@ -1580,7 +1778,7 @@
 
 static void dwt16_prefix(DwGroup& G) {
   G.wg0[0] = 0;
-  for (int i = 0; i < G.n; ++i)
+  for (int i = 0; i < G.ng; ++i)
     G.wg0[i + 1] = G.wg0[i] + ((G.g[i].M + 15) / 16) * ((G.g[i].N + 15) / 16);
 }
 
@@ -1589,6 +1787,27 @@
 static thread_local int64_t g_pre_need = 0;
 
 constexpr size_t kDwdLds = (size_t)2 * 4 * DWG_NT * 64 * sizeof(float4);
+
+static const char* dw_group_name(const DwGroup& G, bool reducer) {
+  static thread_local char buf[2][320];
+  char* b = buf[reducer ? 1 : 0];
+  size_t o = (size_t)snprintf(b, sizeof(buf[0]), "%s", reducer ? "gemm_group_reduce_kernel<gemm_dwd_group_kernel<"
+                                                            : "gemm_dwd_group_kernel<");
+  int seen[kDwGroupMax], ns = 0;
+  for (int i = 0; i < G.n; ++i) {
+    const int c = G.e[i].cls;
+    bool dup = false;
+    for (int j = 0; j < ns; ++j) dup = dup || seen[j] == c;
+    if (dup) continue;
+    seen[ns++] = c;
+    const int mt = c & 7, nt = (c >> 3) & 15;
+    o += (size_t)snprintf(b + o, sizeof(buf[0]) - o, "%s%d%sx%d%s", ns > 1 ? "," : "", mt,
+                          mt == 4 ? ((c >> 7) & 1 ? "v" : "s") : "", nt,
+                          nt >= 4 ? ((c >> 8) & 1 ? "v" : "s") : "");
+  }
+  snprintf(b + o, sizeof(buf[0]) - o, "%s", reducer ? ">>" : ">");
+  return b;
+}
 
 int dw_group_flush(hipStream_t st) {
   g_grp_on = false;
@@ -1601,7 +1820,8 @@
   if (G.x.on && G.x.sq && missed)
     return set_error(SMI_E_ARG, "dw group: a fused sum of squares needs every dW GEMM of the "
                                 "bracket in the group (one ran outside it)");
-  if (G.n == 0 && !pre) {
+  G.n = 0;
+  if (G.ng == 0 && !pre) {
     if (!G.x.on) return SMI_OK;
     if (G.x.sq) return set_error(SMI_E_ARG, "dw group: fused sum of squares over an empty group");
     G.rb0[0] = 0;
@@ -1609,38 +1829,42 @@
     return check_launch("gemm_group_reduce_kernel");
   }
   if (!pre && !G.x.on && use_t16()) {
-    bool small = G.n > 0;
-    for (int i = 0; i < G.n; ++i) small = small && G.g[i].K <= 4 * 16 * T16_MAXC;
+    bool small = G.ng > 0;
+    for (int i = 0; i < G.ng; ++i) small = small && G.g[i].K <= 4 * 16 * T16_MAXC;
     if (small) {
       dwt16_prefix(G);
       const int kslot = ktime_begin(st);
-      hipLaunchKernelGGL(gemm_dwt16_kernel, dim3(G.wg0[G.n]), dim3(kWG), 0, st, G);
+      hipLaunchKernelGGL(gemm_dwt16_kernel, dim3(G.wg0[G.ng]), dim3(kWG), 0, st, G);
       ktime_end(kslot, KT_GEMM_DW, g_grp_flops, st);
       return check_launch("gemm_dwt16_kernel");
     }
   }
   int64_t need = 0;
-  if (G.n > 0) {
-    RC_CHECK(dw_prepare(G, dwd_waves(), dwd_group_slots(kDwdLds), 0, need));
+  if (G.ng > 0) {
+    if (pre && g_pre.ng + G.ng > kDwGemmMax) return set_error(SMI_E_ARG, "dw group: too many GEMMs");
+    RC_CHECK(dw_prepare(G, dwd_waves(), dwd_group_slots(kDwdLds), 0, need,
+                        kDwGroupMax - (pre ? g_pre.n : 0)));
     const int kslot = ktime_begin(st);
     if (dwd_waves() == 8)
       hipLaunchKernelGGL(gemm_dwd_group_kernel<8>, dim3(G.wg0[G.n]), dim3(512), kDwdLds, st, G);
     else
       hipLaunchKernelGGL(gemm_dwd_group_kernel<4>, dim3(G.wg0[G.n]), dim3(256), kDwdLds, st, G);
     ktime_end(kslot, KT_GEMM_DW, g_grp_flops, st);
-    RC_CHECK(check_launch("gemm_dwd_group_kernel"));
+    RC_CHECK(check_launch(dw_group_name(G, false)));
   }
   DwGroup R = G;
   if (pre) {
     R = g_pre;
     R.x = G.x;
     if (R.n + G.n > kDwGroupMax) return set_error(SMI_E_ARG, "dw group: too many entries");
+    for (int i = 0; i < G.ng; ++i) R.g[R.ng + i] = G.g[i];
     for (int i = 0; i < G.n; ++i) {
       const int j = R.n + i;
-      R.g[j] = G.g[i];
-      R.S[j] = G.S[i];
-      R.rb0[j + 1] = R.rb0[j] + (int)(((int64_t)G.g[i].M * G.g[i].N + 64 * red_u() - 1) / (64 * red_u()));
-    }
+      R.e[j] = G.e[i];
+      R.e[j].gi += R.ng;
+      R.rb0[j + 1] = R.rb0[j] + (G.rb0[i + 1] - G.rb0[i]);
+    }
+    R.ng += G.ng;
     R.n += G.n;
     need += g_pre_need;
   }
@@ -1652,7 +1876,7 @@
     hipLaunchKernelGGL(gemm_group_reduce_kernel<1>, dim3(R.rb0[R.n] + (R.x.on ? 1 : 0)), dim3(kWG), 0,
                        st, R);
   ktime_end(rslot, KT_GEMM_REDUCE, (double)need, st);
-  return check_launch("gemm_group_reduce_kernel");
+  return check_launch(dw_group_name(R, true));
 }
 
 static bool use_bwd_dw() {
@@ -1663,7 +1887,7 @@
 int launch_lstm_bwd_dw(const float* dh, const float* gates, const float* cbuf, const float* w_hh,
                        int S, int B, int H, float* dgates, hipStream_t st, const int* skip) {
   const int br = lstm_bwd_q_form(B, H, w_hh);
-  if (!use_bwd_dw() || !g_grp_on || g_pre_on || g_grp.n == 0 || br == 0 || S <= 0 || B <= 0)
+  if (!use_bwd_dw() || !g_grp_on || g_pre_on || g_grp.ng == 0 || br == 0 || S <= 0 || B <= 0)
     return SMI_E_NOFIT;
   int cus = 0, dev = 0;
   (void)hipGetDevice(&dev);
@@ -1671,7 +1895,7 @@
   if (cus - B < 32) return SMI_E_NOFIT;
   DwGroup Ga = g_grp;
   int64_t need = 0;
-  RC_CHECK(dw_prepare(Ga, 8, cus - B, 0, need));
+  RC_CHECK(dw_prepare(Ga, 8, cus - B, 0, need, kDwGroupMax - (kDwGemmMax - Ga.ng)));
   static const bool excl = [] { const char* e = getenv("SMI_BWD_DW_EXCL"); return !(e && e[0] == '0'); }();
   size_t lds = excl ? std::max(kDwdLds, (size_t)84 * 1024) : kDwdLds;
   const size_t stg = (size_t)lstm_bwd_stage_floats(S, H) * 4;
@@ -1700,7 +1924,7 @@
   g_pre_on = true;
   g_pre_need = need;
   workspace_reserve(need);
-  g_grp.n = 0;
+  g_grp.ng = g_grp.n = 0;
   g_grp_flops = 0.0;
   return SMI_OK;
 }
```

After: 3.846 million env-steps/s (median of 6 runs). +2.7%, better.
